# KarolinaBenkova/FEM-FCT-PDECO

Measured on AMD Instinct MI355X. Metric: FCT timesteps/sec (fwd+adj), higher is better.
Workload: dtype f64; 1 GPU; C2 advection_solidbody_FCT_PDECO_finaltime: [-1,1]^2 81x81 P1 (dx=0.025, n=6561), dt=1e-3, 250 fwd + 250 adj FCT steps per cost+gradient evaluation; nodes=6561, num_steps=250, batch_per_gpu=1, parallelism=single trajectory, low_order_solver=jacobi, jacobi_sweeps_max=26, graphs=True, graph_replay=True, kernel_regime=2

## Files before the change

fem-fct-pdeco_amd/csrc/ctx.hip:

```cpp
#include "femfct_internal.h"
#include "build_id.h"
#include "device_utils.h"

#include <dlfcn.h>
#include <stdarg.h>
#include <stdio.h>
#include <stdlib.h>
#include <string.h>
#include <algorithm>
#include <tuple>

int femfct_enqueue_artdiff(femfct_ctx* ctx, const double* K, double* D, int32_t batch);
int femfct_enqueue_spmv(femfct_ctx* ctx, const double* A, const double* x, double alpha, double beta, double* y,
                        int32_t batch);
int femfct_enqueue_cheb(femfct_ctx* ctx, const double* b, double* y_out, int iters, double lmin, double lmax,
                        int32_t batch, bool first_done_in_y1, const double* mdv = nullptr);
int femfct_mesh_release(femfct_ctx* ctx);
int femfct_build_structured_csr(femfct_ctx* ctx);

int femfct_fail(femfct_ctx* ctx, int code, const char* fmt, ...) {
    char buf[1024];
    va_list ap;
    va_start(ap, fmt);
    vsnprintf(buf, sizeof buf, fmt, ap);
    va_end(ap);
    if (ctx) ctx->err = buf;
    return code;
}

namespace {

__global__ void k_scatter_csr_to_ell(int64_t nnz, const int32_t* __restrict__ map, const double* __restrict__ v,
                                     double* __restrict__ ell) {
    int64_t k = (int64_t)blockIdx.x * blockDim.x + threadIdx.x;
    if (k < nnz) ell[map[k]] = v[k];
}

__global__ void k_gather_ell_to_csr(int64_t nnz, const int32_t* __restrict__ map, const double* __restrict__ ell,
                                    double* __restrict__ v) {
    int64_t k = (int64_t)blockIdx.x * blockDim.x + threadIdx.x;
    if (k < nnz) v[k] = ell[map[k]];
}

__global__ void k_mask_popcount(int64_t nbytes, const unsigned long long* __restrict__ mask, unsigned long long* __restrict__ out) {
    __shared__ unsigned long long s[256];
    unsigned long long c = 0;
    const int64_t words = nbytes >> 3;
    for (int64_t k = threadIdx.x; k < words; k += blockDim.x) c += (unsigned long long)__popcll(mask[k]);
    if (threadIdx.x == 0)
        for (int64_t k = words * 8; k < nbytes; ++k) c += (unsigned long long)__popc(reinterpret_cast<const uint8_t*>(mask)[k]);
    s[threadIdx.x] = c;
    __syncthreads();
    for (int o = 128; o > 0; o >>= 1) {
        if ((int)threadIdx.x < o) s[threadIdx.x] += s[threadIdx.x + o];
        __syncthreads();
    }
    if (threadIdx.x == 0) *out = s[0];
}

template <class T>
int dev_alloc(femfct_ctx* ctx, T** p, size_t count) {
    if (*p) { hipFree(*p); *p = nullptr; }
    if (count == 0) return FEMFCT_OK;
    hipError_t e = hipMalloc((void**)p, count * sizeof(T));
    if (e != hipSuccess) {
        *p = nullptr;
        return femfct_fail(ctx, FEMFCT_ERR_NOMEM, "hipMalloc(%zu bytes) failed: %s", count * sizeof(T),
                           hipGetErrorString(e));
    }
    return FEMFCT_OK;
}

template <class T>
void dev_free(T** p) {
    if (*p) hipFree(*p);
    *p = nullptr;
}

}

void femfct_release_pattern(femfct_ctx* ctx) {
    femfct_drop_graphs(ctx);
    dev_free(&ctx->d_cols); dev_free(&ctx->d_tslot); dev_free(&ctx->d_csr2ell); dev_free(&ctx->d_d2v);
    dev_free(&ctx->d_M); dev_free(&ctx->d_Ad); dev_free(&ctx->d_ml);
    dev_free(&ctx->d_L); dev_free(&ctx->d_D); dev_free(&ctx->d_F);
    dev_free(&ctx->d_b); dev_free(&ctx->d_xa); dev_free(&ctx->d_xb);
    dev_free(&ctx->d_du); dev_free(&ctx->d_y0); dev_free(&ctx->d_y1); dev_free(&ctx->d_y2); dev_free(&ctx->d_rdu);
    dev_free(&ctx->d_rp); dev_free(&ctx->d_rm); dev_free(&ctx->d_part); dev_free(&ctx->d_ctl);
    dev_free(&ctx->d_bigpart); ctx->bigpart_count = 0;
    dev_free(&ctx->d_Lmask);
    dev_free(&ctx->d_partk);
    dev_free(&ctx->d_zero);
    dev_free(&ctx->d_rot_check); ctx->rot_om_set = false;
    dev_free(&ctx->d_hA); dev_free(&ctx->d_hN); dev_free(&ctx->d_hrhs); dev_free(&ctx->d_hu);
    dev_free(&ctx->d_hout); dev_free(&ctx->d_hcsr);
    femfct_mesh_release(ctx);
    ctx->h_indptr.clear(); ctx->h_indices.clear(); ctx->h_csr2ell.clear(); ctx->h_cols.clear();
    dev_free(&ctx->d_trAall); ctx->trAall_count = 0;
    dev_free(&ctx->d_lowall); ctx->lowall_count = 0; ctx->low_src = nullptr;
    dev_free(&ctx->d_trA); dev_free(&ctx->d_trN); dev_free(&ctx->d_trRhs); dev_free(&ctx->d_level); dev_free(&ctx->d_log);
    dev_free(&ctx->d_ticket);
    ctx->tr_batch = 0; ctx->tr_steps = 0;
    dev_free(&ctx->d_scratch); ctx->scratch_count = 0;
    dev_free(&ctx->d_ttab); ctx->ttab_count = 0; ctx->h_ttab.clear();
    dev_free(&ctx->d_kry); dev_free(&ctx->d_kry_part); dev_free(&ctx->d_chs_om); dev_free(&ctx->d_chs_scale);
    ctx->chs_om_cap = 0;
    if (ctx->d_kry_ctl) { hipFree(ctx->d_kry_ctl); ctx->d_kry_ctl = nullptr; }
    if (ctx->d_kry_ctl2) { hipFree(ctx->d_kry_ctl2); ctx->d_kry_ctl2 = nullptr; }
    if (ctx->d_klog) { hipFree(ctx->d_klog); ctx->d_klog = nullptr; }
    ctx->kry_batch = 0;
    dev_free(&ctx->d_wscale); ctx->wscale_count = 0;
    dev_free(&ctx->d_zero_traj); ctx->zero_traj_count = 0;
    dev_free(&ctx->d_trMat); dev_free(&ctx->d_trBase); dev_free(&ctx->d_trBase2); dev_free(&ctx->d_trRhs2); dev_free(&ctx->d_trTmp);
    ctx->implicit_cols = false;
    ctx->n = 0; ctx->W = 0; ctx->nnz_csr = 0; ctx->ws_batch = 0; ctx->have_mass = false; ctx->structured = false; ctx->mass_is_mesh = false;
    ctx->sweep_budget = std::min(femfct_ctx().sweep_budget, ctx->max_iters);
    femfct_forget_jacobi_budgets(ctx);
}

void femfct_prof_begin(femfct_ctx* ctx, int cls) {
    if (!ctx->prof_on) return;
    femfct_ctx::ProfRec r;
    r.cls = cls;
    hipEventCreate(&r.a);
    hipEventCreate(&r.b);
    hipEventRecord(r.a, ctx->stream);
    ctx->prof.push_back(r);
}

void femfct_prof_end(femfct_ctx* ctx) {
    if (!ctx->prof_on || ctx->prof.empty()) return;
    hipEventRecord(ctx->prof.back().b, ctx->stream);
}

void femfct_drop_graphs(femfct_ctx* ctx) {
    for (auto& kv : ctx->graphs) hipGraphExecDestroy(kv.second);
    ctx->graphs.clear();
}

int femfct_ensure_workspace(femfct_ctx* ctx, int32_t batch) {
    if (ctx->solver == FEMFCT_SOLVER_BICGSTAB) {
        int rk = femfct_ensure_krylov_ws(ctx, batch);
        if (rk != FEMFCT_OK) return rk;
    }
#ifdef FEMFCT_TUNING
    if (!ctx->d_mesh_trace && getenv("FEMFCT_MESH_TRACE"))
        HIP_TRY(ctx, hipMalloc((void**)&ctx->d_mesh_trace, 16 * sizeof(unsigned long long)));
#endif
    if (!ctx->d_zero && ctx->n > 0) {
        int rz = dev_alloc(ctx, &ctx->d_zero, (size_t)ctx->n);
        if (rz != FEMFCT_OK) return rz;
        HIP_TRY(ctx, hipMemsetAsync(ctx->d_zero, 0, sizeof(double) * ctx->n, ctx->stream));
    }
    if (batch <= ctx->ws_batch) return FEMFCT_OK;
    femfct_drop_graphs(ctx);
    size_t nv = (size_t)batch * ctx->n, nm = nv * ctx->W;
    int rc;
#define A_(p, c) if ((rc = dev_alloc(ctx, &ctx->p, (c))) != FEMFCT_OK) return rc
    A_(d_L, nm + 1); A_(d_D, nm); A_(d_F, nm);
    HIP_TRY(ctx, hipMemsetAsync(ctx->d_L + nm, 0, sizeof(double), ctx->stream));
    A_(d_b, nv); A_(d_xa, nv); A_(d_xb, nv); A_(d_du, nv); A_(d_y0, nv); A_(d_y1, nv); A_(d_y2, nv);
    A_(d_rdu, nv); A_(d_rp, nv); A_(d_rm, nv);
    A_(d_part, (size_t)batch * 4 * FEMFCT_MAX_PARTIALS);
    A_(d_ctl, (size_t)batch);
    A_(d_partk, (size_t)batch * 16 * FEMFCT_MAX_PARTIALS);
    {
        const size_t words = ((size_t)batch * (size_t)ctx->n + 7) / 8 + 1;
        A_(d_Lmask, words);
        HIP_TRY(ctx, hipMemsetAsync(ctx->d_Lmask, 0, words * 8, ctx->stream));
    }
    {
        TilePlan tp;
        ctx->bigpart_count = 0;
        if (femfct_tile_plan(ctx, &tp, false) && femfct_tile_big(ctx, tp)) {
            ctx->bigpart_count = (int64_t)tp.tiles * tp.tiles;
            A_(d_bigpart, (size_t)batch * ctx->bigpart_count);
        }
    }
#undef A_
    HIP_TRY(ctx, hipMemsetAsync(ctx->d_ctl, 0, sizeof(StepCtl) * batch, ctx->stream));
    ctx->ws_batch = batch;
    return FEMFCT_OK;
}

static int fusion_mode(const femfct_ctx* ctx, int* K) {
    TilePlan tp;
    if (femfct_tile_plan(ctx, &tp, false)) {
        *K = tp.K;
        return femfct_tile_big(ctx, tp) ? 1 : 2;
    }
    StripPlan pl;
    if (femfct_strip_plan(ctx, &pl)) { *K = pl.K; return 1; }
    *K = 1;
    return 0;
}

int femfct_fused_k(const femfct_ctx* ctx) {
    int K;
    fusion_mode(ctx, &K);
    return K;
}

int femfct_next_budget(const femfct_ctx* ctx, int worst, bool coarse) {
    int K;
    const int mode = fusion_mode(ctx, &K);
    int b;
    if (mode == 2) b = std::max(worst, 1) + ((coarse || !ctx->exact_iters) ? 0 : 1);
    else if (mode == 1) b = std::max(worst, 1);
    else b = std::max(8, worst + worst / 8 + 2);
    return std::min(ctx->max_iters, b);
}

int femfct_grow_budget(const femfct_ctx* ctx, int budget) {
    int K;
    const int mode = fusion_mode(ctx, &K);
    if (mode == 2) return std::min(ctx->max_iters, budget + 2);
    if (mode == 1) return std::min(ctx->max_iters, budget + K);
    return std::min(ctx->max_iters, budget * 2);
}

int femfct_round_budget(const femfct_ctx* ctx, int b) {
    int K;
    if (fusion_mode(ctx, &K) == 0) b = (b + 3) & ~3;
    if (b < 1) b = 1;
    if (b > ctx->max_iters) b = ctx->max_iters;
    return b;
}

int femfct_install_pattern(femfct_ctx* ctx, int32_t n, int32_t W, const std::vector<int32_t>& cols,
                           const std::vector<uint8_t>& tslot) {
    int rc;
    ctx->n = n;
    ctx->W = W;
    if ((rc = dev_alloc(ctx, &ctx->d_cols, (size_t)W * n)) != FEMFCT_OK) return rc;
    if ((rc = dev_alloc(ctx, &ctx->d_tslot, (size_t)W * n)) != FEMFCT_OK) return rc;
    HIP_TRY(ctx, hipMemcpy(ctx->d_cols, cols.data(), sizeof(int32_t) * W * n, hipMemcpyHostToDevice));
    HIP_TRY(ctx, hipMemcpy(ctx->d_tslot, tslot.data(), sizeof(uint8_t) * W * n, hipMemcpyHostToDevice));
    if ((rc = dev_alloc(ctx, &ctx->d_M, (size_t)W * n)) != FEMFCT_OK) return rc;
    if ((rc = dev_alloc(ctx, &ctx->d_ml, (size_t)n)) != FEMFCT_OK) return rc;
    ctx->h_cols = cols;
    int32_t bwmax = 0;
    for (int32_t s = 1; s < W; ++s)
        for (int32_t i = 0; i < n; ++i) {
            int32_t d = cols[(size_t)s * n + i] - i;
            if (d < 0) d = -d;
            if (d > bwmax) bwmax = d;
        }
    ctx->bandwidth = bwmax;
    if (const char* e = getenv("FEMFCT_STRIPS")) ctx->use_strips = atoi(e) != 0;
    if (const char* e = getenv("FEMFCT_STRIP_K")) ctx->strip_k = atoi(e);
    if (const char* e = getenv("FEMFCT_TILES")) ctx->use_tiles = atoi(e) != 0;
    if (const char* e = getenv("FEMFCT_EXACT")) ctx->exact_iters = atoi(e) != 0;
    if (const char* e = getenv("FEMFCT_FUSE_BUILD")) ctx->fuse_build = atoi(e) != 0;
    if (const char* e = getenv("FEMFCT_PREASSEMBLE")) ctx->preassemble = atoi(e) != 0;
    if (const char* e = getenv("FEMFCT_PREASSEMBLE_MAX_GB")) ctx->preassemble_max_bytes = atof(e) * 1024.0 * 1024.0 * 1024.0;
    if (const char* e = getenv("FEMFCT_PREBUILD_LOW")) ctx->prebuild_low = atoi(e) != 0;
    if (const char* e = getenv("FEMFCT_WG_SLOTS")) ctx->wg_slots = std::max(1, atoi(e));
    if (const char* e = getenv("FEMFCT_DEEP_HALO")) ctx->deep_halo = atoi(e) != 0;
    if (const char* e = getenv("FEMFCT_FUSE_FLUX")) ctx->fuse_flux = atoi(e) != 0;
    if (const char* e = getenv("FEMFCT_FUSE_DUDT")) ctx->fuse_dudt = atoi(e) != 0;
    if (const char* e = getenv("FEMFCT_TILE_LEAN")) ctx->tile_lean = atoi(e) != 0;
    if (const char* e = getenv("FEMFCT_FUSE_END")) ctx->fuse_end = atoi(e) != 0;
    if (const char* e = getenv("FEMFCT_TILE4")) ctx->tile4_mode = atoi(e);
    if (const char* e = getenv("FEMFCT_LMASK")) ctx->l_mask = atoi(e) != 0;
    if (const char* e = getenv("FEMFCT_T4_XCD")) ctx->t4_xcd = atoi(e) != 0;
    if (const char* e = getenv("FEMFCT_T4_WALK")) ctx->t4_walk = atoi(e);
    if (const char* e = getenv("FEMFCT_T4_SNAKE")) ctx->t4_snake = atoi(e) != 0;
    if (const char* e = getenv("FEMFCT_T4_PAIR")) ctx->t4_pair = atoi(e) != 0;
#ifdef FEMFCT_TUNING
    if (const char* e = getenv("FEMFCT_PAIR_SHAPE")) ctx->pair_shape = atoi(e);
    if (const char* e = getenv("FEMFCT_PAIR_PRIO")) ctx->pair_prio = atoi(e);
    if (const char* e = getenv("FEMFCT_PAIR_SPLIT")) ctx->pair_split = std::min(90, std::max(10, atoi(e)));
    if (getenv("FEMFCT_PAIR_TRACE") && !ctx->d_pair_trace) {
        if (hipMalloc((void**)&ctx->d_pair_trace, sizeof(unsigned long long) * (FEMFCT_MAX_PARTIALS * 16 * 5 + 16)) == hipSuccess)
            hipMemset(ctx->d_pair_trace, 0, sizeof(unsigned long long) * (FEMFCT_MAX_PARTIALS * 16 * 5 + 16));
    }
    if (const char* e = getenv("FEMFCT_PAIR_STAGGER_US")) ctx->pair_stagger = (int)(atof(e) * 100.0);
#endif
    if (const char* e = getenv("FEMFCT_DEFER_CHECK")) ctx->defer_check = atoi(e) != 0;
    if (const char* e = getenv("FEMFCT_T4_INT")) ctx->t4_int = atoi(e) != 0;
    if (const char* e = getenv("FEMFCT_T4_WALKERS")) { int v = atoi(e); if (v > 0) ctx->num_cus = v; }
    if (const char* e = getenv("FEMFCT_INLINE_OPS")) ctx->inline_ops = atoi(e) != 0;
    if (const char* e = getenv("FEMFCT_HALF_D")) ctx->half_d = atoi(e) != 0;
    if (const char* e = getenv("FEMFCT_T4_STAGGER_US")) {
        const double us = atof(e);
        int pat = 7;
        if (const char* p = getenv("FEMFCT_T4_STAGGER_PAT")) pat = atoi(p);
        ctx->t4_stagger = us > 0 ? ((int)(us * 100.0) & 0xffffff) | ((pat & 15) << 24) : 0;
    }
    if (const char* e = getenv("FEMFCT_SINGLE_PATCH_BATCH")) { int v = atoi(e); ctx->single_patch_min_batch = v > 0 ? v : (1 << 30); }
    if (const char* e = getenv("FEMFCT_MESH_SOLVE")) ctx->mesh_solve = atoi(e) != 0;
    if (const char* e = getenv("FEMFCT_GEOM_MASS")) ctx->geom_mass = atoi(e) != 0;
    if (const char* e = getenv("FEMFCT_GEOM_ROT")) ctx->geom_rot = atoi(e) != 0;
    if (const char* e = getenv("FEMFCT_FORM_GROUPS")) ctx->form_groups = atoi(e) != 0;
    if (const char* e = getenv("FEMFCT_MESH_STEP")) ctx->mesh_step = atoi(e) != 0;
    if (const char* e = getenv("FEMFCT_MESH_STEP_BATCH")) ctx->mesh_step_min_batch = std::max(1, atoi(e));
    if (const char* e = getenv("FEMFCT_MESH_STEP_BATCH_LARGE")) ctx->mesh_step_min_batch_large = std::max(1, atoi(e));
    if (const char* e = getenv("FEMFCT_T4_DPP")) ctx->t4_dpp = atoi(e) != 0;
    if (const char* e = getenv("FEMFCT_T4_K")) ctx->t4_k = std::min(8, std::max(1, atoi(e)));
    if (const char* e = getenv("FEMFCT_SPECIES_SOLVER")) ctx->species_solver = atoi(e);
    if (const char* e = getenv("FEMFCT_STEPS_PER_GRAPH")) ctx->steps_per_graph = std::max(1, atoi(e));
    return femfct_strip_init(ctx);
}

static int build_csr_map(femfct_ctx* ctx) {
    const int32_t n = ctx->n, W = ctx->W;
    ctx->nnz_csr = ctx->h_indptr[n];
    ctx->h_csr2ell.assign(ctx->nnz_csr, 0);
    for (int32_t i = 0; i < n; ++i) {
        for (int32_t k = ctx->h_indptr[i]; k < ctx->h_indptr[i + 1]; ++k) {
            int32_t j = ctx->h_indices[k];
            int32_t s_found = -1;
            if (j == i) s_found = 0;
            else
                for (int32_t s = 1; s < W; ++s)
                    if (ctx->h_cols[(size_t)s * n + i] == j) { s_found = s; break; }
            if (s_found < 0) return femfct_fail(ctx, FEMFCT_ERR_INVALID, "CSR entry (%d,%d) not in the ELL pattern", i, j);
            ctx->h_csr2ell[k] = (int32_t)((size_t)s_found * n + i);
        }
    }
    int rc;
    if ((rc = dev_alloc(ctx, &ctx->d_csr2ell, (size_t)ctx->nnz_csr)) != FEMFCT_OK) return rc;
    HIP_TRY(ctx, hipMemcpy(ctx->d_csr2ell, ctx->h_csr2ell.data(), sizeof(int32_t) * ctx->nnz_csr, hipMemcpyHostToDevice));
    if ((rc = dev_alloc(ctx, &ctx->d_hcsr, (size_t)ctx->nnz_csr)) != FEMFCT_OK) return rc;
    return FEMFCT_OK;
}

extern "C" {

int femfct_abi_version(void) { return FEMFCT_ABI_VERSION; }
const char* femfct_build_id(void) { return FEMFCT_BUILD_ID; }

}

bool femfct_profiler_attached() {
    for (const char* name : {"librocprofiler-sdk.so.1", "librocprofiler-sdk.so"}) {
        if (void* h = dlopen(name, RTLD_LAZY | RTLD_NOLOAD)) {
            dlclose(h);
            return true;
        }
    }
    return false;
}

extern "C" {

int femfct_create(femfct_ctx** out, int device_id) {
    if (!out) return FEMFCT_ERR_INVALID;
    *out = nullptr;
    int count = 0;
    if (hipGetDeviceCount(&count) != hipSuccess || count <= 0) return FEMFCT_ERR_HIP;
    if (device_id < 0 || device_id >= count) return FEMFCT_ERR_INVALID;
    if (hipSetDevice(device_id) != hipSuccess) return FEMFCT_ERR_HIP;
    femfct_ctx* ctx = new (std::nothrow) femfct_ctx();
    if (!ctx) return FEMFCT_ERR_NOMEM;
    ctx->device = device_id;
    {
        int cus = 0;
        if (hipDeviceGetAttribute(&cus, hipDeviceAttributeMultiprocessorCount, device_id) == hipSuccess && cus > 0) ctx->num_cus = cus;
    }
    if (hipStreamCreateWithFlags(&ctx->stream, hipStreamNonBlocking) != hipSuccess) {
        delete ctx;
        return FEMFCT_ERR_HIP;
    }
    const char* pg = getenv("FEMFCT_PROFILER_GRAPHS");
    ctx->profiler_graphs_ok = pg && atoi(pg) != 0;
    if (!ctx->profiler_graphs_ok && femfct_profiler_attached()) ctx->graphs_blocked = true;
    *out = ctx;
    return FEMFCT_OK;
}

int femfct_graph_replay_active(const femfct_ctx* ctx, int* active_host) {
    if (!ctx || !active_host) return FEMFCT_ERR_INVALID;
    *active_host = (ctx->use_graphs && !ctx->prof_on && !ctx->graphs_blocked) ? 1 : 0;
    return FEMFCT_OK;
}

int femfct_rotation_derived(const femfct_ctx* ctx, int* derived_host) {
    if (!ctx || !derived_host) return FEMFCT_ERR_INVALID;
    *derived_host = ctx->last_rot_geom ? 1 : 0;
    return FEMFCT_OK;
}

int femfct_destroy(femfct_ctx* ctx) {
    if (!ctx) return FEMFCT_OK;
    hipSetDevice(ctx->device);
    hipStreamSynchronize(ctx->stream);
    if (ctx->d_pair_trace) {
        if (const char* path = getenv("FEMFCT_PAIR_TRACE")) {
            std::vector<unsigned long long> h((size_t)FEMFCT_MAX_PARTIALS * 16 * 5 + 16);
            if (hipMemcpy(h.data(), ctx->d_pair_trace, h.size() * sizeof(unsigned long long), hipMemcpyDeviceToHost) == hipSuccess)
                if (FILE* f = fopen(path, "wb")) { fwrite(h.data(), sizeof(unsigned long long), h.size(), f); fclose(f); }
        }
        hipFree(ctx->d_pair_trace);
        ctx->d_pair_trace = nullptr;
    }
    femfct_release_pattern(ctx);
    hipStreamDestroy(ctx->stream);
    delete ctx;
    return FEMFCT_OK;
}

const char* femfct_last_error(const femfct_ctx* ctx) { return ctx ? ctx->err.c_str() : "null context"; }

int femfct_synchronize(femfct_ctx* ctx) {
    FEMFCT_ENTER(ctx);
    ARG_TRY(ctx, ctx, "null ctx");
    HIP_TRY(ctx, hipStreamSynchronize(ctx->stream));
    return FEMFCT_OK;
}

void* femfct_stream(femfct_ctx* ctx) { return ctx ? (void*)ctx->stream : nullptr; }

int femfct_set_solver(femfct_ctx* ctx, int solver, double rel_tol, int max_iters) {
    FEMFCT_ENTER(ctx);
    ARG_TRY(ctx, ctx, "null ctx");
    ARG_TRY(ctx, solver == FEMFCT_SOLVER_JACOBI || solver == FEMFCT_SOLVER_BICGSTAB, "unknown solver");
    ARG_TRY(ctx, rel_tol > 0 && rel_tol < 1 && max_iters >= 1, "bad tolerance / iteration cap");
    ctx->solver = solver;
    ctx->solver_user = solver;
    femfct_forget_bicgstab_handovers(ctx);
    ctx->rel_tol = rel_tol;
    ctx->max_iters = max_iters;
    if (ctx->sweep_budget > max_iters) ctx->sweep_budget = max_iters;
    femfct_forget_jacobi_budgets(ctx);
    femfct_drop_graphs(ctx);
    return FEMFCT_OK;
}

int femfct_set_fusion(femfct_ctx* ctx, int strips, int tiles) {
    FEMFCT_ENTER(ctx);
    ARG_TRY(ctx, ctx, "null ctx");
    HIP_TRY(ctx, hipStreamSynchronize(ctx->stream));
    ctx->use_strips = strips != 0;
    ctx->use_tiles = tiles != 0;
    femfct_drop_graphs(ctx);
    femfct_forget_jacobi_budgets(ctx);
    ctx->ws_batch = 0;
    return FEMFCT_OK;
}

int femfct_kernel_regime(const femfct_ctx* ctx, int32_t batch) {
    if (!ctx || ctx->n <= 0) return -1;
    if (femfct_mesh_step_wanted(ctx, batch)) return FEMFCT_REGIME_MESH;
    if (femfct_tile4_wanted(ctx, batch)) return FEMFCT_REGIME_PATCH64;
    TilePlan tp;
    if (ctx->use_strips && femfct_tile_plan(ctx, &tp, true, 0, batch)) return FEMFCT_REGIME_TILE32;
    StripPlan sp;
    if (femfct_strip_plan(ctx, &sp)) return FEMFCT_REGIME_STRIPS;
    return FEMFCT_REGIME_ROWS;
}

int femfct_patch_walkers(const femfct_ctx* ctx, int32_t batch, int32_t sweeps) {
    if (!ctx || ctx->n <= 0 || batch < 1 || !femfct_tile4_wanted(ctx, batch) || femfct_single_patch(ctx, batch)) return 0;
    return femfct_tile4_walkers(ctx, femfct_tile4_halo(ctx, sweeps > 0 ? sweeps : 36), batch, false);
}

int femfct_launch_info(const femfct_ctx* ctx, int32_t* out4_host) {
    if (!ctx || !out4_host) return FEMFCT_ERR_INVALID;
    for (int k = 0; k < 4; ++k) out4_host[k] = ctx->last_launch[k];
    return FEMFCT_OK;
}

int femfct_lowop_nonzero_fraction(femfct_ctx* ctx, double* fraction_host) {
    FEMFCT_ENTER(ctx);
    ARG_TRY(ctx, fraction_host, "null argument");
    *fraction_host = 1.0;
    if (!ctx->d_Lmask || ctx->n <= 0 || !ctx->l_mask || !femfct_tile4_wanted(ctx, 1) || !ctx->t4_dpp ||
        ctx->solver != FEMFCT_SOLVER_JACOBI)
        return FEMFCT_OK;
    unsigned long long* d_cnt = nullptr;
    HIP_TRY(ctx, hipMalloc((void**)&d_cnt, sizeof(unsigned long long)));
    hipLaunchKernelGGL(k_mask_popcount, dim3(1), dim3(256), 0, ctx->stream, (int64_t)ctx->n, ctx->d_Lmask + 1, d_cnt);
    unsigned long long cnt = 0;
    HIP_TRY(ctx, hipMemcpyAsync(&cnt, d_cnt, sizeof cnt, hipMemcpyDeviceToHost, ctx->stream));
    HIP_TRY(ctx, hipStreamSynchronize(ctx->stream));
    hipFree(d_cnt);
    *fraction_host = (double)cnt / (6.0 * (double)ctx->n);
    return FEMFCT_OK;
}

int femfct_set_graphs(femfct_ctx* ctx, int enable) {
    FEMFCT_ENTER(ctx);
    ARG_TRY(ctx, ctx, "null ctx");
    ctx->use_graphs = enable != 0;
    if (!enable) femfct_drop_graphs(ctx);
    return FEMFCT_OK;
}

int femfct_set_profiling(femfct_ctx* ctx, int enable) {
    FEMFCT_ENTER(ctx);
    ARG_TRY(ctx, ctx, "null ctx");
    HIP_TRY(ctx, hipStreamSynchronize(ctx->stream));
    for (auto& r : ctx->prof) { hipEventDestroy(r.a); hipEventDestroy(r.b); }
    ctx->prof.clear();
    ctx->prof_on = enable != 0;
    return FEMFCT_OK;
}

int femfct_profile_report(femfct_ctx* ctx, double* total_ms_host, int32_t* launches_host, int32_t n_classes) {
    FEMFCT_ENTER(ctx);
    ARG_TRY(ctx, ctx && total_ms_host && launches_host && n_classes >= KC_COUNT, "need >= 8 classes");
    HIP_TRY(ctx, hipStreamSynchronize(ctx->stream));
    for (int k = 0; k < n_classes; ++k) { total_ms_host[k] = 0.0; launches_host[k] = 0; }
    for (auto& r : ctx->prof) {
        float ms = 0.f;
        if (hipEventElapsedTime(&ms, r.a, r.b) == hipSuccess) {
            total_ms_host[r.cls] += ms;
            launches_host[r.cls] += 1;
        }
        hipEventDestroy(r.a);
        hipEventDestroy(r.b);
    }
    ctx->prof.clear();
    return FEMFCT_OK;
}

int femfct_malloc(femfct_ctx* ctx, void** dev_ptr, size_t bytes) {
    FEMFCT_ENTER(ctx);
    ARG_TRY(ctx, ctx && dev_ptr, "null argument");
    HIP_TRY(ctx, hipSetDevice(ctx->device));
    hipError_t e = hipMalloc(dev_ptr, bytes ? bytes : 8);
    if (e != hipSuccess) return femfct_fail(ctx, FEMFCT_ERR_NOMEM, "hipMalloc(%zu) failed: %s", bytes, hipGetErrorString(e));
    return FEMFCT_OK;
}
int femfct_free(femfct_ctx* ctx, void* p) {
    FEMFCT_ENTER(ctx);
    ARG_TRY(ctx, ctx, "null ctx");
    HIP_TRY(ctx, hipStreamSynchronize(ctx->stream));
    HIP_TRY(ctx, hipFree(p));
    return FEMFCT_OK;
}
int femfct_memcpy_h2d(femfct_ctx* ctx, void* d, const void* h, size_t bytes) {
    FEMFCT_ENTER(ctx);
    ARG_TRY(ctx, ctx && (bytes == 0 || (d && h)), "null argument");
    HIP_TRY(ctx, hipMemcpyAsync(d, h, bytes, hipMemcpyHostToDevice, ctx->stream));
    HIP_TRY(ctx, hipStreamSynchronize(ctx->stream));
    return FEMFCT_OK;
}
int femfct_memcpy_d2h(femfct_ctx* ctx, void* h, const void* d, size_t bytes) {
    FEMFCT_ENTER(ctx);
    ARG_TRY(ctx, ctx && (bytes == 0 || (d && h)), "null argument");
    HIP_TRY(ctx, hipMemcpyAsync(h, d, bytes, hipMemcpyDeviceToHost, ctx->stream));
    HIP_TRY(ctx, hipStreamSynchronize(ctx->stream));
    return FEMFCT_OK;
}
int femfct_memcpy_d2d(femfct_ctx* ctx, void* d, const void* s, size_t bytes) {
    FEMFCT_ENTER(ctx);
    ARG_TRY(ctx, ctx && (bytes == 0 || (d && s)), "null argument");
    HIP_TRY(ctx, hipMemcpyAsync(d, s, bytes, hipMemcpyDeviceToDevice, ctx->stream));
    return FEMFCT_OK;
}
int femfct_memset0(femfct_ctx* ctx, void* d, size_t bytes) {
    FEMFCT_ENTER(ctx);
    ARG_TRY(ctx, ctx && (bytes == 0 || d), "null argument");
    HIP_TRY(ctx, hipMemsetAsync(d, 0, bytes, ctx->stream));
    return FEMFCT_OK;
}

int femfct_set_pattern_csr(femfct_ctx* ctx, int32_t n, const int32_t* indptr, const int32_t* indices) {
    FEMFCT_ENTER(ctx);
    ARG_TRY(ctx, ctx && indptr && indices && n > 0, "null/empty pattern");
    HIP_TRY(ctx, hipSetDevice(ctx->device));
    HIP_TRY(ctx, hipStreamSynchronize(ctx->stream));
    femfct_release_pattern(ctx);
    ARG_TRY(ctx, indptr[0] == 0, "indptr[0] must be 0");
    int32_t W = 1;
    for (int32_t i = 0; i < n; ++i) {
        ARG_TRY(ctx, indptr[i + 1] >= indptr[i], "indptr not monotone");
        int32_t len = 0;
        bool diag = false;
        for (int32_t k = indptr[i]; k < indptr[i + 1]; ++k) {
            int32_t j = indices[k];
            ARG_TRY(ctx, j >= 0 && j < n, "column index out of range");
            if (j == i) diag = true; else ++len;
        }
        ARG_TRY(ctx, diag, "pattern must contain the full diagonal");
        W = std::max(W, len + 1);
    }
    if (W > FEMFCT_MAX_W) return femfct_fail(ctx, FEMFCT_ERR_INVALID, "row with %d entries exceeds FEMFCT_MAX_W=%d", W, FEMFCT_MAX_W);
    std::vector<int32_t> cols((size_t)W * n);
    std::vector<uint8_t> tslot((size_t)W * n);
    for (int32_t s = 0; s < W; ++s)
        for (int32_t i = 0; i < n; ++i) { cols[(size_t)s * n + i] = i; tslot[(size_t)s * n + i] = (uint8_t)s; }
    for (int32_t i = 0; i < n; ++i) {
        int32_t s = 1;
        for (int32_t k = indptr[i]; k < indptr[i + 1]; ++k) {
            int32_t j = indices[k];
            if (j == i) continue;
            for (int32_t q = 1; q < s; ++q)
                ARG_TRY(ctx, cols[(size_t)q * n + i] != j, "duplicate column in a row");
            cols[(size_t)s * n + i] = j;
            ++s;
        }
    }
    for (int32_t i = 0; i < n; ++i)
        for (int32_t s = 1; s < W; ++s) {
            int32_t j = cols[(size_t)s * n + i];
            if (j == i) continue;
            int32_t ts = -1;
            for (int32_t q = 1; q < W; ++q)
                if (cols[(size_t)q * n + j] == i) { ts = q; break; }
            if (ts < 0) return femfct_fail(ctx, FEMFCT_ERR_INVALID, "pattern not symmetric: (%d,%d) has no transpose", i, j);
            tslot[(size_t)s * n + i] = (uint8_t)ts;
        }
    int rc = femfct_install_pattern(ctx, n, W, cols, tslot);
    if (rc != FEMFCT_OK) return rc;
    ctx->h_indptr.assign(indptr, indptr + n + 1);
    ctx->h_indices.assign(indices, indices + indptr[n]);
    return build_csr_map(ctx);
}

int32_t femfct_n(const femfct_ctx* ctx) { return ctx ? ctx->n : 0; }
int32_t femfct_ell_width(const femfct_ctx* ctx) { return ctx ? ctx->W : 0; }

int femfct_get_ell_cols(femfct_ctx* ctx, int32_t* cols_host) {
    FEMFCT_ENTER(ctx);
    ARG_TRY(ctx, ctx && cols_host && ctx->n > 0, "no pattern");
    memcpy(cols_host, ctx->h_cols.data(), sizeof(int32_t) * ctx->h_cols.size());
    return FEMFCT_OK;
}


static int need_csr_map(femfct_ctx* ctx) {
    ARG_TRY(ctx, ctx && ctx->n > 0, "no pattern registered");
    if (ctx->d_csr2ell) return FEMFCT_OK;
    if (ctx->structured) {
        int rc = femfct_build_structured_csr(ctx);
        if (rc != FEMFCT_OK) return rc;
        return build_csr_map(ctx);
    }
    return femfct_fail(ctx, FEMFCT_ERR_INVALID, "no CSR pattern");
}

int femfct_csr_to_ell(femfct_ctx* ctx, const double* csr_vals_host, double* ell_dev) {
    FEMFCT_ENTER(ctx);
    int rc = need_csr_map(ctx);
    if (rc != FEMFCT_OK) return rc;
    ARG_TRY(ctx, csr_vals_host && ell_dev, "null argument");
    HIP_TRY(ctx, hipMemcpyAsync(ctx->d_hcsr, csr_vals_host, sizeof(double) * ctx->nnz_csr, hipMemcpyHostToDevice, ctx->stream));
    HIP_TRY(ctx, hipMemsetAsync(ell_dev, 0, sizeof(double) * ctx->W * ctx->n, ctx->stream));
    int bs = 256;
    hipLaunchKernelGGL(k_scatter_csr_to_ell, dim3((unsigned)((ctx->nnz_csr + bs - 1) / bs)), dim3(bs), 0, ctx->stream,
                       ctx->nnz_csr, ctx->d_csr2ell, ctx->d_hcsr, ell_dev);
    HIP_TRY(ctx, hipStreamSynchronize(ctx->stream));
    return FEMFCT_OK;
}

int femfct_ell_to_csr(femfct_ctx* ctx, const double* ell_dev, double* csr_vals_host) {
    FEMFCT_ENTER(ctx);
    int rc = need_csr_map(ctx);
    if (rc != FEMFCT_OK) return rc;
    ARG_TRY(ctx, csr_vals_host && ell_dev, "null argument");
    int bs = 256;
    hipLaunchKernelGGL(k_gather_ell_to_csr, dim3((unsigned)((ctx->nnz_csr + bs - 1) / bs)), dim3(bs), 0, ctx->stream,
                       ctx->nnz_csr, ctx->d_csr2ell, ell_dev, ctx->d_hcsr);
    HIP_TRY(ctx, hipMemcpyAsync(csr_vals_host, ctx->d_hcsr, sizeof(double) * ctx->nnz_csr, hipMemcpyDeviceToHost, ctx->stream));
    HIP_TRY(ctx, hipStreamSynchronize(ctx->stream));
    return FEMFCT_OK;
}

int femfct_set_mass(femfct_ctx* ctx, const double* M_csr_vals_host, const double* ml_host) {
    FEMFCT_ENTER(ctx);
    ARG_TRY(ctx, ctx && ctx->n > 0, "no pattern registered");
    ARG_TRY(ctx, M_csr_vals_host && ml_host, "null argument");
    HIP_TRY(ctx, hipStreamSynchronize(ctx->stream));
    femfct_drop_graphs(ctx);
    int rc = femfct_csr_to_ell(ctx, M_csr_vals_host, ctx->d_M);
    if (rc != FEMFCT_OK) return rc;
    HIP_TRY(ctx, hipMemcpy(ctx->d_ml, ml_host, sizeof(double) * ctx->n, hipMemcpyHostToDevice));
    ctx->have_mass = true;
    ctx->mass_is_mesh = false;
    return FEMFCT_OK;
}

const double* femfct_mass_ell(const femfct_ctx* ctx) { return ctx && ctx->have_mass ? ctx->d_M : nullptr; }
const double* femfct_stiffness_ell(const femfct_ctx* ctx) { return ctx ? ctx->d_Ad : nullptr; }
const double* femfct_lumped_mass(const femfct_ctx* ctx) { return ctx && ctx->have_mass ? ctx->d_ml : nullptr; }

static int launch_step(femfct_ctx* ctx, const double* A, const double* N, int32_t nshared, const double* rhs,
                       const double* u_n, double dt, double* u_out, int32_t batch) {
    const int budget = femfct_round_budget(ctx, ctx->sweep_budget);
    femfct_ctx::GraphKey key{(uint64_t)1, key_bits(A), key_bits(N), key_bits(rhs), key_bits(u_n), key_bits(u_out),
                             key_bits(nshared), key_bits(batch), key_bits((int32_t)budget), key_bits(dt),
                             key_bits(ctx->rel_tol)};
    return femfct_run_graph(ctx, key, [&]() {
        return femfct_enqueue_step(ctx, A, N, nshared, rhs, u_n, dt, u_out, batch, budget);
    });
}

int femfct_fct_step(femfct_ctx* ctx, const double* A_ell, const double* N_ell, int32_t N_shared, const double* rhs,
                    const double* u_n, double dt, double* u_out, int32_t batch) {
    FEMFCT_ENTER(ctx);
    ARG_TRY(ctx, ctx && ctx->n > 0, "no pattern registered");
    ARG_TRY(ctx, ctx->have_mass, "mass matrix not set (femfct_set_mass / femfct_set_mesh_square)");
    ARG_TRY(ctx, A_ell && u_n && u_out, "null argument");
    ARG_TRY(ctx, batch >= 1 && dt > 0, "batch must be >= 1 and dt > 0");
    int rc = femfct_ensure_workspace(ctx, batch);
    if (rc != FEMFCT_OK) return rc;
    return launch_step(ctx, A_ell, N_ell, N_shared, rhs, u_n, dt, u_out, batch);
}

int femfct_last_step_info(femfct_ctx* ctx, femfct_step_info* info, int32_t batch) {
    FEMFCT_ENTER(ctx);
    ARG_TRY(ctx, ctx && info && batch >= 1 && batch <= ctx->ws_batch, "bad argument");
    std::vector<StepCtl> h(batch);
    HIP_TRY(ctx, hipMemcpyAsync(h.data(), ctx->d_ctl, sizeof(StepCtl) * batch, hipMemcpyDeviceToHost, ctx->stream));
    HIP_TRY(ctx, hipStreamSynchronize(ctx->stream));
    int worst = 0;
    for (int b = 0; b < batch; ++b) {
        info[b].flags = h[b].flags;
        info[b].solver_iters = h[b].iters;
        info[b].solver_resid = h[b].resid;
        info[b].min_rowsum = h[b].min_rowsum;
        worst = std::max(worst, h[b].iters);
    }
    bool short_of = false;
    for (int b = 0; b < batch; ++b) short_of = short_of || (h[b].flags & FEMFCT_FLAG_SOLVER_BUDGET);
    ctx->sweep_budget = short_of ? femfct_grow_budget(ctx, femfct_round_budget(ctx, ctx->sweep_budget))
                                 : femfct_next_budget(ctx, worst);
    return FEMFCT_OK;
}

int femfct_fct_step_host(femfct_ctx* ctx, const double* A_csr, const double* N_csr, const double* rhs,
                         const double* u_n, double dt, double* u_out, femfct_step_info* info) {
    FEMFCT_ENTER(ctx);
    ARG_TRY(ctx, ctx && ctx->n > 0, "no pattern registered");
    ARG_TRY(ctx, A_csr && u_n && u_out, "null argument");
    int rc;
    const size_t n = ctx->n, nm = n * ctx->W;
    if (!ctx->d_hA) {
        if ((rc = dev_alloc(ctx, &ctx->d_hA, nm)) != FEMFCT_OK) return rc;
        if ((rc = dev_alloc(ctx, &ctx->d_hN, nm)) != FEMFCT_OK) return rc;
        if ((rc = dev_alloc(ctx, &ctx->d_hrhs, n)) != FEMFCT_OK) return rc;
        if ((rc = dev_alloc(ctx, &ctx->d_hu, n)) != FEMFCT_OK) return rc;
        if ((rc = dev_alloc(ctx, &ctx->d_hout, n)) != FEMFCT_OK) return rc;
    }
    if ((rc = femfct_csr_to_ell(ctx, A_csr, ctx->d_hA)) != FEMFCT_OK) return rc;
    if (N_csr && (rc = femfct_csr_to_ell(ctx, N_csr, ctx->d_hN)) != FEMFCT_OK) return rc;
    if (rhs) HIP_TRY(ctx, hipMemcpyAsync(ctx->d_hrhs, rhs, sizeof(double) * n, hipMemcpyHostToDevice, ctx->stream));
    HIP_TRY(ctx, hipMemcpyAsync(ctx->d_hu, u_n, sizeof(double) * n, hipMemcpyHostToDevice, ctx->stream));
    femfct_step_info local;
    for (;;) {
        rc = femfct_fct_step(ctx, ctx->d_hA, N_csr ? ctx->d_hN : nullptr, 0, rhs ? ctx->d_hrhs : nullptr, ctx->d_hu,
                             dt, ctx->d_hout, 1);
        if (rc != FEMFCT_OK) return rc;
        const int used_budget = femfct_round_budget(ctx, ctx->sweep_budget);
        if ((rc = femfct_last_step_info(ctx, &local, 1)) != FEMFCT_OK) return rc;
        if (!(local.flags & FEMFCT_FLAG_SOLVER_BUDGET)) break;
        if (used_budget >= ctx->max_iters || !(local.solver_resid < INFINITY))
            return femfct_fail(ctx, FEMFCT_ERR_NOT_CONVERGED,
                               "low-order solve: residual %.3e after %d sweeps (tol %.1e)", local.solver_resid,
                               local.solver_iters, ctx->rel_tol);
        ctx->sweep_budget = femfct_grow_budget(ctx, used_budget);
    }
    if (info) *info = local;
    HIP_TRY(ctx, hipMemcpyAsync(u_out, ctx->d_hout, sizeof(double) * n, hipMemcpyDeviceToHost, ctx->stream));
    HIP_TRY(ctx, hipStreamSynchronize(ctx->stream));
    return FEMFCT_OK;
}

int femfct_chebsi(femfct_ctx* ctx, const double* b_dev, double* y_dev, int32_t cheb_iter, double lmin, double lmax,
                  int32_t batch) {
    FEMFCT_ENTER(ctx);
    ARG_TRY(ctx, ctx && ctx->n > 0 && ctx->have_mass, "mass matrix not set");
    ARG_TRY(ctx, b_dev && y_dev && cheb_iter >= 1 && batch >= 1 && lmin + lmax != 0, "bad argument");
    int rc = femfct_ensure_workspace(ctx, batch);
    if (rc != FEMFCT_OK) return rc;
    return femfct_enqueue_cheb(ctx, b_dev, y_dev, cheb_iter, lmin, lmax, batch, false);
}

int femfct_chebsi_md(femfct_ctx* ctx, const double* b_dev, double* y_dev, const double* md_dev, int32_t cheb_iter,
                     double lmin, double lmax, int32_t batch) {
    FEMFCT_ENTER(ctx);
    ARG_TRY(ctx, ctx && ctx->n > 0 && ctx->have_mass, "mass matrix not set");
    ARG_TRY(ctx, b_dev && y_dev && md_dev && cheb_iter >= 1 && batch == 1 && lmin + lmax != 0, "bad argument");
    int rc = femfct_ensure_workspace(ctx, batch);
    if (rc != FEMFCT_OK) return rc;
    return femfct_enqueue_cheb(ctx, b_dev, y_dev, cheb_iter, lmin, lmax, batch, false, md_dev);
}

int femfct_artificial_diffusion(femfct_ctx* ctx, const double* K_ell, double* D_ell, int32_t batch) {
    FEMFCT_ENTER(ctx);
    ARG_TRY(ctx, ctx && ctx->n > 0, "no pattern registered");
    ARG_TRY(ctx, K_ell && D_ell && batch >= 1, "bad argument");
    return femfct_enqueue_artdiff(ctx, K_ell, D_ell, batch);
}

int femfct_spmv(femfct_ctx* ctx, const double* mat_ell, const double* x_dev, double alpha, double beta, double* y_dev,
                int32_t batch) {
    FEMFCT_ENTER(ctx);
    ARG_TRY(ctx, ctx && ctx->n > 0, "no pattern registered");
    ARG_TRY(ctx, mat_ell && x_dev && y_dev && batch >= 1, "bad argument");
    return femfct_enqueue_spmv(ctx, mat_ell, x_dev, alpha, beta, y_dev, batch);
}

}
```

fem-fct-pdeco_amd/csrc/femfct_internal.h:

```cpp
#pragma once

#include <hip/hip_runtime.h>
#include <stdint.h>
#include <string.h>
#include <string>
#include <vector>
#include <map>
#include <tuple>

#include "../../include/femfct.h"

#define FEMFCT_MAX_W 16
#ifndef FEMFCT_MAX_PARTIALS
#define FEMFCT_MAX_PARTIALS 2048
#endif

struct StepCtl {
    int32_t flags;
    int32_t iters;
    int32_t done;
    int32_t parity;
    double  resid;
    double  bnorm;
    double  min_rowsum;
    double  rs[2];
    double  pad;
};

enum SweepKind {
    SWEEP_SOLIDBODY_FORWARD = 2, SWEEP_SOLIDBODY_ADJOINT = 3,
    SWEEP_NONLINEAR_FORWARD = 10, SWEEP_NONLINEAR_ADJOINT = 11,
    SWEEP_SCHNAK_FORWARD = 12, SWEEP_SCHNAK_ADJOINT = 13,
    SWEEP_CHTXS_FORWARD = 14, SWEEP_CHTXS_ADJOINT = 15,
    SWEEP_NONLINEAR_ADJOINT_ALLTIME = 16,
};

struct SweepKindState {
    int budget = 48;
    int good = 0;
    int fail = 0;
    int mesh_cap = 0;
    int cheb_budget = 40;
    int bicg_budget = 40;
    bool full_rows = false;
    bool low_bicg = false;
    bool cheb_off = false;
};

struct femfct_ctx {
    int device = 0;
    hipStream_t stream = nullptr;
    std::string err;

    int32_t n = 0;
    int32_t W = 0;
    int64_t nnz_csr = 0;
    int32_t* d_cols = nullptr;
    uint8_t* d_tslot = nullptr;
    int32_t* d_csr2ell = nullptr;
    std::vector<int32_t> h_indptr, h_indices, h_csr2ell, h_cols;
    bool structured = false;
    bool mass_is_mesh = false;
    double a1 = 0, a2 = 0, h = 0;
    int32_t n_cells = 0, N = 0, order = 0;
    int32_t* d_d2v = nullptr;

    double* d_M = nullptr;
    double* d_Ad = nullptr;
    double* d_ml = nullptr;
    bool have_mass = false;

    int solver = FEMFCT_SOLVER_JACOBI;
    int solver_user = FEMFCT_SOLVER_JACOBI;
    double rel_tol = 1e-13;
    int max_iters = 400;
    int sweep_budget = 48;
    std::map<int, SweepKindState> kinds;
    bool use_graphs = true;
    bool graphs_blocked = false;
    int graph_captures = 0;
    bool profiler_graphs_ok = false;
    int32_t steps_per_graph = 50;
    bool use_strips = true;
    bool use_tiles = true;
    bool mesh_solve = true;
    bool mesh_solve_attr[8] = {false, false, false, false, false, false, false, false};
    int single_patch_min_batch = 8;
    bool form_groups = true;
    bool geom_rot = true;
    double rot_om = 0.0;
    bool rot_om_set = false;
    int* d_rot_check = nullptr;
    bool last_rot_geom = false;
    bool geom_mass = true;
    bool t4_dpp = true;
    int t4_k = 8;
    int t4_snake = 1;
    bool t4_pair = true;
    int pair_stagger = 0;
    int32_t last_launch[4] = {0, 0, 0, 0};
    unsigned long long* d_pair_trace = nullptr;
    int pair_prio = 0, pair_split = 50;
    int pair_shape = 5;
    bool pair_rows = false;
    bool mesh_step = true;
    int mesh_step_min_batch = 1;
    int mesh_step_min_batch_large = 64;
    bool mesh_step_attr[6] = {false, false, false, false, false, false};
    double* d_zero = nullptr;
    unsigned long long* d_mesh_trace = nullptr;
    int defer_check = 1;
    int t4_int = 1;
    int t4_walk = 1;
    int num_cus = 256;
    int t4_xcd = 0;
    int t4_stagger = 600 | (7 << 24);
    int tile4_mode = 1;
    bool fuse_end = true;
    bool fuse_build = true;
    int wg_slots = 256;
    bool deep_halo = true;
    bool fuse_flux = true;
    bool fuse_dudt = true;
    int tile_lean = 1;
    bool exact_iters = false;
    int32_t bandwidth = 0;
    int32_t strip_k = 0;
    bool implicit_cols = false;

    int32_t ws_batch = 0;
    double *d_L = nullptr, *d_D = nullptr, *d_F = nullptr;
    double *d_b = nullptr, *d_xa = nullptr, *d_xb = nullptr;
    double *d_du = nullptr, *d_y0 = nullptr, *d_y1 = nullptr, *d_y2 = nullptr, *d_rdu = nullptr;
    double *d_rp = nullptr, *d_rm = nullptr;
    double *d_part = nullptr;
    StepCtl* d_ctl = nullptr;
    double* d_partk = nullptr;
    double* d_bigpart = nullptr;
    unsigned long long* d_Lmask = nullptr;
    bool half_d = true;
    bool inline_ops = true;
    bool l_mask = true;
    int64_t bigpart_count = 0;
    double *d_hA = nullptr, *d_hN = nullptr, *d_hrhs = nullptr, *d_hu = nullptr, *d_hout = nullptr, *d_hcsr = nullptr;

    typedef std::vector<uint64_t> GraphKey;
    std::map<GraphKey, hipGraphExec_t> graphs;

    int32_t tr_batch = 0, tr_steps = 0;
    double* d_trAall = nullptr;
    size_t trAall_count = 0;
    bool preassemble = true;
    double preassemble_max_bytes = 16.0 * 1024 * 1024 * 1024;
    bool prebuild_low = true;
    double* d_lowall = nullptr;
    size_t lowall_count = 0, low_doff = 0;
    const double* low_src = nullptr;
    double low_dt = 0.0;
    double *d_trA = nullptr, *d_trN = nullptr, *d_trRhs = nullptr;
    int32_t* d_level = nullptr;
    StepCtl* d_log = nullptr;
    unsigned* d_ticket = nullptr;
    int level_bias = 0, ord_bias = 0, rep_total = 1;
    bool rep_last = true;
    int end_req_delta = 0;
    bool end_req_krylov = false, end_fused = false;
    std::vector<StepCtl> h_log;
    int32_t log_steps = 0, log_batch = 0;

    bool prof_on = false;
    struct ProfRec { int cls; hipEvent_t a, b; };
    std::vector<ProfRec> prof;

    int32_t kry_batch = 0;
    double* d_kry = nullptr;
    double* d_kry_part = nullptr;
    void* d_kry_ctl = nullptr;
    void* d_kry_ctl2 = nullptr;
    double kry_tol = 1e-13;
    int kry_max_iters = 2000;
    int kry_budget = 40;
    void* d_klog = nullptr;
    int species_solver = 0;
    double* d_chs_om = nullptr;
    double* d_chs_scale = nullptr;
    int chs_om_cap = 0;
    std::vector<char> h_klog;
    double *d_trMat = nullptr, *d_trBase = nullptr, *d_trBase2 = nullptr;
    double *d_trRhs2 = nullptr, *d_trTmp = nullptr;
    double* d_wscale = nullptr;
    size_t wscale_count = 0;
    double* d_zero_traj = nullptr;
    size_t zero_traj_count = 0;

    double* d_scratch = nullptr;
    size_t scratch_count = 0;
    int32_t* d_ttab = nullptr;
    size_t ttab_count = 0;
    std::vector<int32_t> h_ttab;
};

int femfct_fail(femfct_ctx* ctx, int code, const char* fmt, ...);
#define HIP_TRY(ctx, expr)                                                          \
    do {                                                                            \
        hipError_t _e = (expr);                                                     \
        if (_e != hipSuccess)                                                       \
            return femfct_fail((ctx), FEMFCT_ERR_HIP, "%s failed: %s (%s:%d)", #expr, \
                               hipGetErrorString(_e), __FILE__, __LINE__);          \
    } while (0)
#define ARG_TRY(ctx, cond, msg)                                                     \
    do {                                                                            \
        if (!(cond)) return femfct_fail((ctx), FEMFCT_ERR_INVALID, "%s", msg);      \
    } while (0)

#define FEMFCT_ENTER(ctx)                                                           \
    do {                                                                            \
        if (!(ctx)) return FEMFCT_ERR_INVALID;                                      \
        HIP_TRY((ctx), hipSetDevice((ctx)->device));                                \
    } while (0)

int femfct_ensure_workspace(femfct_ctx* ctx, int32_t batch);
int femfct_ensure_krylov_ws(femfct_ctx* ctx, int32_t batch);
void femfct_drop_graphs(femfct_ctx* ctx);
void femfct_release_pattern(femfct_ctx* ctx);
int femfct_round_budget(const femfct_ctx* ctx, int b);
#define FEMFCT_INTERNAL __attribute__((visibility("hidden")))
FEMFCT_INTERNAL void femfct_forget_jacobi_budgets(femfct_ctx* ctx);
FEMFCT_INTERNAL void femfct_forget_bicgstab_handovers(femfct_ctx* ctx);
FEMFCT_INTERNAL void femfct_forget_cheb_off(femfct_ctx* ctx);
FEMFCT_INTERNAL int femfct_ensure_scratch(femfct_ctx* ctx, size_t doubles);
FEMFCT_INTERNAL void femfct_enqueue_reduce_levels(femfct_ctx* ctx, int32_t batch, int levels, int G, const double* partial,
                                                  int trapezoid, double scale, int accumulate, double* out_dev);

static inline uint64_t key_bits(const void* p) { return (uint64_t)(uintptr_t)p; }
static inline uint64_t key_bits(double d) { uint64_t u; memcpy(&u, &d, 8); return u; }
static inline uint64_t key_bits(int64_t v) { return (uint64_t)v; }
static inline uint64_t key_bits(int32_t v) { return (uint64_t)(int64_t)v; }
template <class F>
int femfct_run_graph(femfct_ctx* ctx, const femfct_ctx::GraphKey& key, F&& enqueue);

static inline bool femfct_tiles_usable(const femfct_ctx* ctx) {
    return ctx->use_strips && ctx->use_tiles && ctx->implicit_cols && ctx->W == 7;
}

struct StripPlan { int K, R, bw, rpt, S; };
bool femfct_strip_plan(const femfct_ctx* ctx, StripPlan* pl);
int femfct_strip_init(femfct_ctx* ctx);
int femfct_enqueue_strip_jacobi(femfct_ctx* ctx, const StripPlan& pl, const double* L, const double* b, double* xa,
                                double* xb, int launch, int g_build, int32_t batch);
int femfct_enqueue_strip_cheb(femfct_ctx* ctx, const StripPlan& pl, const double* b, const double* in_mid,
                              const double* in_old, double* y_out, int k_first, int k_last, const double* omegas,
                              double md_scale, double* bufA0, double* bufA1, double* bufB0, double* bufB1,
                              int32_t batch);

struct TilePlan { int tiles, K, H; };
bool femfct_tile_plan(const femfct_ctx* ctx, TilePlan* pl, bool need_partials = true, int budget = 0, int batch = 1);
bool femfct_tile_big(const femfct_ctx* ctx, const TilePlan& pl);
bool femfct_cheb_flux_fusable(const femfct_ctx* ctx, int32_t batch);
bool femfct_geom_mass(const femfct_ctx* ctx);
int femfct_enqueue_tile_build_jacobi(femfct_ctx* ctx, const TilePlan& pl, struct MatRef A, const double* Nm, int32_t nshared,
                                     struct VecRef rhs, int64_t rhs_bstride, struct VecRef u_n, int64_t u_bstride, double dt,
                                     int32_t batch, bool pre = false);
int femfct_enqueue_low_seq(femfct_ctx* ctx, const double* A, double* L, double* D, int32_t entries, double dt);
int femfct_enqueue_tile_jacobi(femfct_ctx* ctx, const TilePlan& pl, const double* L, const double* b, double* xa,
                               double* xb, int launch, int g_build, int32_t batch, bool last, int bn_launch = 0, int defer = 0);
__attribute__((visibility("hidden"))) void femfct_launch_reduce_resid(femfct_ctx* ctx, int64_t count, int launch, int32_t batch);
int femfct_enqueue_tile_dudt_cheb(femfct_ctx* ctx, struct MatRef A, struct VecRef rhs, int64_t rhs_bstride, double* ulow,
                                  int budget_units, int part_count, int iters_per_unit, int exact_k, int iters,
                                  const double* omegas, double md_scale, int32_t batch, int* tail_first = nullptr);
int femfct_enqueue_tile_cheb(femfct_ctx* ctx, const TilePlan& pl, const double* b, const double* in_mid,
                             const double* in_old, double* y_out, int k_first, int k_last, const double* omegas,
                             double md_scale, double* bufA0, double* bufA1, double* bufB0, double* bufB1, int32_t batch,
                             const struct ChebIO* io = nullptr);
int femfct_enqueue_tile_cheb_flux_limit(femfct_ctx* ctx, const double* b, const double* in_mid, const double* in_old,
                                        int k_first, int k_last, const double* omegas, double md_scale, struct MatRef D,
                                        const double* ulow, double dt, struct VecRef out, int64_t out_bstride, int32_t batch,
                                        bool fuse_end);
int femfct_enqueue_tile_flux_limit(femfct_ctx* ctx, const double* D, const double* ulow, const double* du, double dt,
                                   struct VecRef out, int64_t out_bstride, int32_t batch, bool* fuse_end_io, int half_d = 0);

bool femfct_tile4_wanted(const femfct_ctx* ctx, int32_t batch);
bool femfct_single_patch(const femfct_ctx* ctx, int32_t batch);
int femfct_tile4_tiles(const femfct_ctx* ctx, int H = 8);
int femfct_tile4_halo(const femfct_ctx* ctx, int sweeps);
int femfct_tile4_walkers(const femfct_ctx* ctx, int H, int32_t batch, bool pair);
bool femfct_jacobi_pair_wanted(const femfct_ctx* ctx, int H, int32_t batch, bool have_lmask, bool assume_upwind_rows = false);
int femfct_tile4_init(femfct_ctx* ctx);
int femfct_enqueue_tile4_jacobi(femfct_ctx* ctx, const double* L, const double* b, double* xa, double* xb, int launch,
                                int g_build, int32_t batch, int H = 8, int K = 8, int check_every = 0,
                                const uint8_t* lmask = nullptr);
int femfct_enqueue_tile4_cheb(femfct_ctx* ctx, const double* b, const double* in_mid, const double* in_old, double* y_out,
                              int k_first, int k_last, const double* omegas, double md_scale, double* bufA0, double* bufA1,
                              double* bufB0, double* bufB1, int32_t batch,
                              const struct ChebIO* io = nullptr);

bool femfct_rotation_is_geometric(femfct_ctx* ctx, const double* Arot, double* om_out);
bool femfct_jacobi_plan(const femfct_ctx* ctx, int budget, int batch, int* K, int* launches);
bool femfct_mesh_step_wanted(const femfct_ctx* ctx, int32_t batch, bool have_nm = false);
int femfct_enqueue_mesh_step(femfct_ctx* ctx, struct MatRef A, const double* Nm, int32_t nshared, struct VecRef rhs,
                             int64_t rhs_bstride, struct VecRef u_n, int64_t u_bstride, double dt, struct VecRef u_out,
                             int64_t out_bstride, int32_t batch, int32_t budget, bool fuse_end);
int femfct_fused_k(const femfct_ctx* ctx);
int femfct_next_budget(const femfct_ctx* ctx, int worst_iters, bool coarse = false);
int femfct_grow_budget(const femfct_ctx* ctx, int budget);

enum { KC_BUILD_LOW = 0, KC_JACOBI, KC_DUDT_RHS, KC_CHEB, KC_FLUX, KC_LIMIT, KC_ASSEMBLE, KC_OTHER, KC_COUNT };
void femfct_prof_begin(femfct_ctx* ctx, int cls);
void femfct_prof_end(femfct_ctx* ctx);

struct LaunchGeom { dim3 grid; dim3 block; };
LaunchGeom femfct_geom(const femfct_ctx* ctx, int32_t batch);

int femfct_enqueue_step(femfct_ctx* ctx, const double* A, const double* N, int32_t nshared,
                        const double* rhs, const double* u_n, double dt, double* u_out,
                        int32_t batch, int32_t budget);

bool femfct_profiler_attached();

template <class F>
int femfct_run_graph(femfct_ctx* ctx, const femfct_ctx::GraphKey& key, F&& enqueue) {
    if (!ctx->use_graphs || ctx->prof_on || ctx->graphs_blocked) return enqueue();
    auto it = ctx->graphs.find(key);
    if (it == ctx->graphs.end()) {
        if (!ctx->profiler_graphs_ok && femfct_profiler_attached()) {
            ctx->graphs_blocked = true;
            return enqueue();
        }
        if (ctx->graphs.size() > 64) femfct_drop_graphs(ctx);
        ++ctx->graph_captures;
        hipGraph_t graph = nullptr;
        HIP_TRY(ctx, hipStreamBeginCapture(ctx->stream, hipStreamCaptureModeThreadLocal));
        int rc = enqueue();
        hipError_t e = hipStreamEndCapture(ctx->stream, &graph);
        if (rc != FEMFCT_OK) { if (graph) hipGraphDestroy(graph); return rc; }
        if (e != hipSuccess) return femfct_fail(ctx, FEMFCT_ERR_HIP, "hipStreamEndCapture: %s", hipGetErrorString(e));
        hipGraphExec_t exec = nullptr;
        e = hipGraphInstantiate(&exec, graph, nullptr, nullptr, 0);
        hipGraphDestroy(graph);
        if (e != hipSuccess) return femfct_fail(ctx, FEMFCT_ERR_HIP, "hipGraphInstantiate: %s", hipGetErrorString(e));
        it = ctx->graphs.emplace(key, exec).first;
    }
    HIP_TRY(ctx, hipGraphLaunch(it->second, ctx->stream));
    return FEMFCT_OK;
}
```

fem-fct-pdeco_amd/csrc/kernels_tile32.hip:

```cpp
#include "femfct_internal.h"
#include "device_utils.h"
#include "solve_ctl.h"
#include "forms.h"
#include "step_end.h"
#include "sweep_common.h"

#include <math.h>

#define TILE_T 16
#define TILE_H 8
#define TILE_L 32
#define TILE_LD 33
#define TILE_HMAX 13

namespace {

struct TileGeom {
    int lx, ly, gx, gy, i;
    bool inside, owned;
    int kvalid;
    int nb[6];
    int self;
};

template <int T = TILE_T, int H = TILE_H, int PL = TILE_L>
__device__ __forceinline__ TileGeom tile_geom(int N) {
    static_assert(T + 2 * H == PL, "patch edge = tile + 2 halos");
    constexpr int PLD = PL + 1;
    TileGeom g;
    g.lx = threadIdx.x % PL;
    g.ly = threadIdx.x / PL;
    const int x0 = blockIdx.x * T - H, y0 = blockIdx.y * T - H;
    g.gx = x0 + g.lx;
    g.gy = y0 + g.ly;
    g.inside = g.gx >= 0 && g.gx < N && g.gy >= 0 && g.gy < N;
    g.i = g.inside ? g.gy * N + g.gx : 0;
    g.owned = g.inside && g.lx >= H && g.lx < H + T && g.ly >= H && g.ly < H + T;
    int kv = 1 << 20;
    if (x0 > 0) kv = min(kv, g.lx);
    if (x0 + PL - 1 < N - 1) kv = min(kv, PL - 1 - g.lx);
    if (y0 > 0) kv = min(kv, g.ly);
    if (y0 + PL - 1 < N - 1) kv = min(kv, PL - 1 - g.ly);
    g.kvalid = g.inside ? kv : 0;
    const int dx[6] = {1, 1, 0, -1, -1, 0}, dy[6] = {0, 1, 1, 0, -1, -1};
    g.self = g.ly * PLD + g.lx;
#pragma unroll
    for (int s = 0; s < 6; ++s) {
        int nx = min(max(g.lx + dx[s], 0), PL - 1), ny = min(max(g.ly + dy[s], 0), PL - 1);
        g.nb[s] = ny * PLD + nx;
    }
    return g;
}

template <int H>
__device__ __forceinline__ int tile_dist(const TileGeom& g) {
    constexpr int T = TILE_L - 2 * H;
    const int ddx = max(max(H - g.lx, g.lx - (H + T - 1)), 0), ddy = max(max(H - g.ly, g.ly - (H + T - 1)), 0);
    return max(ddx, ddy);
}

struct LeanAddr {
    const double* n0[6];
    double* me0;
};

__device__ __forceinline__ LeanAddr lean_addr(double (*bufs)[TILE_L * TILE_LD], const TileGeom& g) {
    LeanAddr a;
    a.me0 = &bufs[0][g.self];
#pragma unroll
    for (int s = 0; s < 6; ++s) a.n0[s] = &bufs[0][g.nb[s]];
    return a;
}

template <int BUF, int LAST>
__device__ __forceinline__ void lean_jacobi_sweep(const LeanAddr& a, bool live, bool owned, const double* lv, double dg,
                                                  double rdg, double bv, double& xo, double& rmax) {
    constexpr int RD = BUF * TILE_L * TILE_LD, WR = (1 - BUF) * TILE_L * TILE_LD;
    if (live) {
        double acc = bv;
#pragma unroll
        for (int s = 0; s < 6; ++s) acc = fma(-lv[s], a.n0[s][RD], acc);
        if (LAST && owned) rmax = nan_max(rmax, fabs(acc - dg * xo));
        xo = acc * rdg;
        a.me0[WR] = xo;
    }
    __syncthreads();
}

__device__ __forceinline__ double lean_jacobi(const LeanAddr& a, int klive, int K, bool owned, const double* lv, double dg,
                                              double rdg, double bv, double xi, double& rmax) {
    double xo = xi;
    int k = 0;
    for (; k + 2 < K; k += 2) {
        lean_jacobi_sweep<0, 0>(a, k < klive, owned, lv, dg, rdg, bv, xo, rmax);
        lean_jacobi_sweep<1, 0>(a, k + 1 < klive, owned, lv, dg, rdg, bv, xo, rmax);
    }
    if (k + 1 < K) {
        lean_jacobi_sweep<0, 0>(a, k < klive, owned, lv, dg, rdg, bv, xo, rmax);
        lean_jacobi_sweep<1, 1>(a, k + 1 < klive, owned, lv, dg, rdg, bv, xo, rmax);
    } else if (k < K) {
        lean_jacobi_sweep<0, 1>(a, k < klive, owned, lv, dg, rdg, bv, xo, rmax);
    }
    return xo;
}

template <int BUF>
__device__ __forceinline__ void lean_cheb_iter(const LeanAddr& a, bool live, const double* mv, double md, double rmd, double bv,
                                               double wk, double& ym, double& yo) {
    constexpr int RD = BUF * TILE_L * TILE_LD, WR = (1 - BUF) * TILE_L * TILE_LD;
    if (live) {
        double acc = md * ym;
#pragma unroll
        for (int s = 0; s < 6; ++s) acc = fma(mv[s], a.n0[s][RD], acc);
        const double z = (bv - acc) * rmd;
        const double yn = wk * (z + ym - yo) + yo;
        yo = ym;
        ym = yn;
        a.me0[WR] = yn;
    }
    __syncthreads();
}

template <int H, int EXACT, int BIG, int LEAN>
__global__ void __launch_bounds__(STRIP_T)
k_tile_jacobi(int n, int N, const double* __restrict__ L_, const double* __restrict__ b_, double* __restrict__ xa_,
              double* __restrict__ xb_, double* __restrict__ part, StepCtl* __restrict__ ctl_, int launch, int K,
              int g_build, double rel_tol, double* __restrict__ bigpart, double* __restrict__ partk, int bn_launch,
              int defer) {
    constexpr int W = 7;
    __shared__ double xs[2][TILE_L * TILE_LD];
    __shared__ double smem[96];
    const int bz = blockIdx.z;
    StepCtl* ctl = ctl_ + bz;
    if (!defer && ctl->done) return;
    double* p = part + (int64_t)bz * 4 * FEMFCT_MAX_PARTIALS;
    const int nwg = gridDim.x * gridDim.y, wg = blockIdx.y * gridDim.x + blockIdx.x;
    double bnorm;
    double rmax_prev = 0.0;
    bool have_rmax = false;
    if (defer) {
        bnorm = 0.0;
    } else if (launch == bn_launch) {
        double rsmin = INFINITY;
        bnorm = 0.0;
        if (!BIG && launch > 0 && g_build == nwg) {
            const double* pr = p + ((launch - 1) & 1) * FEMFCT_MAX_PARTIALS;
            for (int k = threadIdx.x; k < nwg; k += blockDim.x) {
                bnorm = nan_max(bnorm, p[2 * FEMFCT_MAX_PARTIALS + k]);
                rmax_prev = nan_max(rmax_prev, pr[k]);
                rsmin = nan_min(rsmin, p[3 * FEMFCT_MAX_PARTIALS + k]);
            }
            block_reduce_max_max_min(bnorm, rmax_prev, rsmin, smem);
            have_rmax = true;
        } else {
            bnorm = reduce_partials(p + 2 * FEMFCT_MAX_PARTIALS, g_build, OpMax(), 0.0, smem);
            rsmin = reduce_partials(p + 3 * FEMFCT_MAX_PARTIALS, g_build, OpMin(), INFINITY, smem);
        }
        if (wg == 0 && threadIdx.x == 0) {
            ctl->bnorm = bnorm;
            ctl->min_rowsum = rsmin;
            if (!(rsmin > 0.0)) ctl->flags |= FEMFCT_FLAG_MMATRIX_ROWSUM;
        }
    } else {
        bnorm = ctl->bnorm;
    }
    if (launch > 0 && !defer) {
        double rmax = have_rmax ? rmax_prev
                      : BIG   ? ctl->rs[(launch - 1) & 1]
                              : reduce_partials(p + ((launch - 1) & 1) * FEMFCT_MAX_PARTIALS, nwg, OpMax(), 0.0, smem);
        if (rmax <= rel_tol * bnorm) {
            if (wg == 0 && threadIdx.x == 0) {
                ctl->done = 1; ctl->parity = launch & 1; ctl->iters = launch * K; ctl->flags |= FEMFCT_FLAG_COARSE_ITERS;
                ctl->resid = bnorm != 0.0 ? rmax / bnorm : 0.0;
            }
            return;
        }
    }
    const int64_t moff = (int64_t)bz * W * n, voff = (int64_t)bz * n;
    const double* L = L_ + moff;
    const double* xin = ((launch & 1) ? xb_ : xa_) + voff;
    double* xout = ((launch & 1) ? xa_ : xb_) + voff;
    const TileGeom g = tile_geom<TILE_L - 2 * H, H>(N);
    double lv[W - 1], dg = 1.0, rdg = 1.0, bv = 0.0, xi = 0.0;
#pragma unroll
    for (int s = 0; s < W - 1; ++s) lv[s] = 0.0;
    if (g.inside) {
        dg = L[g.i];
        rdg = 1.0 / dg;
#pragma unroll
        for (int s = 1; s < W; ++s) lv[s - 1] = L[(int64_t)s * n + g.i];
        bv = b_[voff + g.i];
        xi = xin[g.i];
    }
    xs[0][g.self] = xi;
    if (LEAN) xs[1][g.self] = xi;
    __syncthreads();
    double rmax = 0.0;
    int cur = 0;
    [[maybe_unused]] double xo = xi;
    [[maybe_unused]] const int klive = min(g.kvalid, K - tile_dist<H>(g));
    [[maybe_unused]] const LeanAddr a = lean_addr(xs, g);
    if (!EXACT) {
        if constexpr (LEAN) xo = lean_jacobi(a, klive, K, g.owned, lv, dg, rdg, bv, xi, rmax);
        else
        for (int k = 0; k < K; ++k) {
            const double* c = xs[cur];
            double xn = c[g.self];
            if (k < g.kvalid) {
                double acc = bv;
#pragma unroll
                for (int s = 0; s < W - 1; ++s) acc = fma(-lv[s], c[g.nb[s]], acc);
                if (k == K - 1 && g.owned) rmax = nan_max(rmax, fabs(acc - dg * xn));
                xn = acc * rdg;
            }
            xs[cur ^ 1][g.self] = xn;
            __syncthreads();
            cur ^= 1;
        }
    } else {
        double rk[H];
#pragma unroll
        for (int k = 0; k < H; ++k) {
            rk[k] = 0.0;
            if (k < K) {
                if constexpr (LEAN) {
                    const int rd = (k & 1) * TILE_L * TILE_LD, wr = ((k + 1) & 1) * TILE_L * TILE_LD;
                    if (k < klive) {
                        double acc = bv;
#pragma unroll
                        for (int s = 0; s < W - 1; ++s) acc = fma(-lv[s], a.n0[s][rd], acc);
                        if (g.owned) rk[k] = fabs(acc - dg * xo);
                        if (k == K - 1) rmax = nan_max(rmax, rk[k]);
                        xo = acc * rdg;
                        a.me0[wr] = xo;
                    }
                    __syncthreads();
                    continue;
                }
                const double* c = xs[cur];
                double xn = c[g.self];
                if (k < g.kvalid) {
                    double acc = bv;
#pragma unroll
                    for (int s = 0; s < W - 1; ++s) acc = fma(-lv[s], c[g.nb[s]], acc);
                    if (g.owned) rk[k] = fabs(acc - dg * xn);
                    if (k == K - 1) rmax = nan_max(rmax, rk[k]);
                    xn = acc * rdg;
                }
                xs[cur ^ 1][g.self] = xn;
                __syncthreads();
                cur ^= 1;
            }
        }
        __shared__ double sk[H][STRIP_T / WAVE];
        const int wid = threadIdx.x / WAVE, lane = threadIdx.x % WAVE;
#pragma unroll
        for (int k = 0; k < H; ++k) {
            double v = wave_reduce(rk[k], OpMax());
            if (lane == 0) sk[k][wid] = v;
        }
        __syncthreads();
        if (threadIdx.x < H) {
            double v = 0.0;
            for (int w = 0; w < STRIP_T / WAVE; ++w) v = nan_max(v, sk[threadIdx.x][w]);
            partk[((int64_t)bz * 16 + threadIdx.x) * FEMFCT_MAX_PARTIALS + wg] = v;
        }
    }
    if (g.owned) xout[g.i] = LEAN ? xo : xs[cur][g.self];
    rmax = block_reduce(rmax, OpMax(), 0.0, smem);
    if (threadIdx.x == 0) {
        if (BIG) bigpart[(int64_t)bz * nwg + wg] = rmax;
        else if (defer) partk[((int64_t)bz * 16 + launch) * FEMFCT_MAX_PARTIALS + wg] = rmax;
        else p[(launch & 1) * FEMFCT_MAX_PARTIALS + wg] = rmax;
    }
}

template <int H, int PRE, int LEAN>
__global__ void __launch_bounds__(STRIP_T)
k_tile_build_jacobi(int n, int N, MatRef A_ref, const double* __restrict__ N_, int nshared,
                    VecRef rhs_ref, int64_t rhs_bstride, VecRef u_ref, int64_t u_bstride,
                    const double* __restrict__ ml, double dt, double* __restrict__ L_, double* __restrict__ D_,
                    double* __restrict__ b_, double* __restrict__ xb_, double* __restrict__ part,
                    StepCtl* __restrict__ ctl_, int K) {
    constexpr int W = 7;
    __shared__ double xs[2][TILE_L * TILE_LD];
    __shared__ double as[PRE ? 1 : 3][TILE_L * TILE_LD];
    __shared__ double smem[96];
    const int bz = blockIdx.z;
    const int wg = blockIdx.y * gridDim.x + blockIdx.x;
    double* p = part + (int64_t)bz * 4 * FEMFCT_MAX_PARTIALS;
    if (wg == 0 && threadIdx.x == 0) {
        StepCtl* c = ctl_ + bz;
        c->flags = 0; c->iters = 0; c->done = 0; c->parity = 0; c->resid = 0.0; c->bnorm = 0.0;
        c->min_rowsum = 0.0;
    }
    const int64_t moff = (int64_t)bz * W * n, voff = (int64_t)bz * n;
    const double* A = mat_ptr(A_ref, bz);
    const double* Nm = N_ ? N_ + (nshared ? 0 : moff) : nullptr;
    const double* rhs = vec_ptr(rhs_ref);
    if (rhs) rhs += bz * rhs_bstride;
    const double* u = vec_ptr(u_ref) + bz * u_bstride;
    const TileGeom g = tile_geom<TILE_L - 2 * H, H>(N);
    double lv[W - 1], dv[W - 1], dsum = 0.0, rs = 0.0;
    double dg = 1.0, rdg = 1.0, bv = 0.0, xi = 0.0;
    if constexpr (PRE) {
#pragma unroll
        for (int s = 0; s < W - 1; ++s) lv[s] = 0.0;
        if (g.inside) {
            dg = A[g.i];
#pragma unroll
            for (int s = 1; s < W; ++s) lv[s - 1] = A[(int64_t)s * n + g.i];
        }
#pragma unroll
        for (int s = 0; s < W - 1; ++s) rs += lv[s];
        if (g.inside) {
            const double mli = ml[g.i];
            rs += dg;
            rdg = 1.0 / dg;
            xi = u[g.i];
            bv = mli * xi + (rhs ? dt * rhs[g.i] : 0.0);
        }
    } else {
        const int dx[6] = {1, 1, 0, -1, -1, 0}, dy[6] = {0, 1, 1, 0, -1, -1};
        bool ex[W - 1];
#pragma unroll
        for (int s = 0; s < W - 1; ++s) {
            const int nx = g.gx + dx[s], ny = g.gy + dy[s];
            ex[s] = g.inside && nx >= 0 && nx < N && ny >= 0 && ny < N;
        }
        double av[W - 1], at[W - 1], a0 = 0.0;
#pragma unroll
        for (int s = 0; s < W - 1; ++s) av[s] = 0.0;
        if (g.inside) {
            a0 = A[g.i];
#pragma unroll
            for (int s = 1; s < W; ++s) av[s - 1] = A[(int64_t)s * n + g.i];
        }
#pragma unroll
        for (int s = 0; s < 3; ++s) as[s][g.self] = av[s + 3];
        __syncthreads();
#pragma unroll
        for (int s = 0; s < 3; ++s) at[s] = as[s][g.nb[s]];
        __syncthreads();
#pragma unroll
        for (int s = 0; s < 3; ++s) as[s][g.self] = av[s];
        __syncthreads();
#pragma unroll
        for (int s = 3; s < 6; ++s) at[s] = as[s - 3][g.nb[s]];
#pragma unroll
        for (int s = 0; s < W - 1; ++s) {
            const double a = av[s];
            const double d = ex[s] ? fmax(0.0, fmax(a, at[s])) : 0.0;
            dsum += d;
            double l = dt * (a - d);
            if (Nm && g.inside) l += dt * Nm[(int64_t)(s + 1) * n + g.i];
            lv[s] = l;
            dv[s] = d;
            rs += l;
        }
        if (g.inside) {
            const double mli = ml[g.i];
            double ld = mli + dt * (a0 + dsum);
            if (Nm) ld += dt * Nm[g.i];
            rs += ld;
            dg = ld;
            rdg = 1.0 / dg;
            xi = u[g.i];
            bv = mli * xi + (rhs ? dt * rhs[g.i] : 0.0);
        }
    }
    double bmax = 0.0, rsmin = INFINITY;
    if (g.owned) {
        double* L = L_ + moff;
        L[g.i] = dg;
#pragma unroll
        for (int s = 1; s < W; ++s) L[(int64_t)s * n + g.i] = lv[s - 1];
        if constexpr (!PRE) {
            double* D = D_ + moff;
            D[g.i] = -dsum;
#pragma unroll
            for (int s = 1; s < W; ++s) D[(int64_t)s * n + g.i] = dv[s - 1];
        }
        b_[voff + g.i] = bv;
        bmax = fabs(bv);
        rsmin = rs;
    }
    xs[0][g.self] = xi;
    if (LEAN) xs[1][g.self] = xi;
    __syncthreads();
    double rmax = 0.0;
    int cur = 0;
    [[maybe_unused]] double xo = xi;
    if constexpr (LEAN) xo = lean_jacobi(lean_addr(xs, g), min(g.kvalid, K - tile_dist<H>(g)), K, g.owned, lv, dg, rdg, bv, xi, rmax);
    else
    for (int k = 0; k < K; ++k) {
        const double* c = xs[cur];
        double xn = c[g.self];
        if (k < g.kvalid) {
            double acc = bv;
#pragma unroll
            for (int s = 0; s < W - 1; ++s) acc = fma(-lv[s], c[g.nb[s]], acc);
            if (k == K - 1 && g.owned) rmax = nan_max(rmax, fabs(acc - dg * xn));
            xn = acc * rdg;
        }
        xs[cur ^ 1][g.self] = xn;
        __syncthreads();
        cur ^= 1;
    }
    if (g.owned) xb_[voff + g.i] = LEAN ? xo : xs[cur][g.self];
    block_reduce_max_max_min(rmax, bmax, rsmin, smem);
    if (threadIdx.x == 0) {
        p[wg] = rmax;
        p[2 * FEMFCT_MAX_PARTIALS + wg] = bmax;
        p[3 * FEMFCT_MAX_PARTIALS + wg] = rsmin;
    }
}

__global__ void __launch_bounds__(256)
k_low_seq(int n, int N, const double* __restrict__ A_, const double* __restrict__ ml, double dt, double* __restrict__ L_,
          double* __restrict__ D_) {
    constexpr int W = 7;
    const int64_t off = (int64_t)blockIdx.y * W * n;
    const double* A = A_ + off;
    double* L = L_ + off;
    double* D = D_ + off;
    const int dx[6] = {1, 1, 0, -1, -1, 0}, dy[6] = {0, 1, 1, 0, -1, -1};
    for (int i = blockIdx.x * blockDim.x + threadIdx.x; i < n; i += gridDim.x * blockDim.x) {
        const int gx = i % N, gy = i / N;
        double av[W - 1], at[W - 1];
        bool ex[W - 1];
        const double a0 = A[i];
#pragma unroll
        for (int s = 0; s < W - 1; ++s) {
            const int nx = gx + dx[s], ny = gy + dy[s];
            ex[s] = nx >= 0 && nx < N && ny >= 0 && ny < N;
            av[s] = A[(int64_t)(s + 1) * n + i];
            at[s] = ex[s] ? A[(int64_t)(s < 3 ? s + 4 : s - 2) * n + ny * N + nx] : 0.0;
        }
        double dsum = 0.0;
#pragma unroll
        for (int s = 0; s < W - 1; ++s) {
            const double a = av[s];
            const double d = ex[s] ? fmax(0.0, fmax(a, at[s])) : 0.0;
            dsum += d;
            L[(int64_t)(s + 1) * n + i] = dt * (a - d);
            D[(int64_t)(s + 1) * n + i] = d;
        }
        L[i] = ml[i] + dt * (a0 + dsum);
        D[i] = -dsum;
    }
}

__global__ void __launch_bounds__(STRIP_T)
k_reduce_resid(const double* __restrict__ bigpart, int64_t count, StepCtl* __restrict__ ctl_, int launch) {
    __shared__ double smem[32];
    const int bz = blockIdx.x;
    if (ctl_[bz].done) return;
    const double* q = bigpart + (int64_t)bz * count;
    double v = 0.0;
    for (int64_t k = threadIdx.x; k < count; k += blockDim.x) v = nan_max(v, q[k]);
    v = block_reduce(v, OpMax(), 0.0, smem);
    if (threadIdx.x == 0) ctl_[bz].rs[launch & 1] = v;
}

template <int H, int LEAN>
__global__ void __launch_bounds__(STRIP_T)
k_tile_cheb(int n, int N, const double* __restrict__ M, const double* __restrict__ b_, const double* __restrict__ ymid_,
            const double* __restrict__ yold_, double* __restrict__ omid_, double* __restrict__ oold_, int K,
            CheOmegas om, double md_scale, ChebIO cio) {
    constexpr int W = 7;
    __shared__ double ys[LEAN ? 2 : 3][TILE_L * TILE_LD];
    const int64_t voff = (int64_t)blockIdx.z * n;
    if (cio.mat) M = cio.mat + (int64_t)blockIdx.z * cio.mat_bs;
    if (cio.scale_dev) md_scale = cio.scale_dev[blockIdx.z];
    const double* omd = cio.om_dev ? cio.om_dev + (int64_t)blockIdx.z * cio.om_bs + cio.k0 : nullptr;
    if (cio.mid_ref.base) ymid_ = vec_ptr(cio.mid_ref) + (int64_t)blockIdx.z * cio.mid_bs - voff;
    if (cio.out_ref.base) omid_ = const_cast<double*>(vec_ptr(cio.out_ref)) + (int64_t)blockIdx.z * cio.out_bs - voff;
    const TileGeom g = tile_geom<TILE_L - 2 * H, H>(N);
    double mv[W - 1], md = 1.0, rmd = 1.0, bv = 0.0, ym = 0.0, yo = 0.0;
#pragma unroll
    for (int s = 0; s < W - 1; ++s) mv[s] = 0.0;
    if (g.inside) {
        md = M[g.i];
        rmd = 1.0 / (md_scale * md);
#pragma unroll
        for (int s = 1; s < W; ++s) mv[s - 1] = M[(int64_t)s * n + g.i];
        bv = b_[voff + g.i];
        if (ymid_) ym = ymid_[voff + g.i];
        if (yold_) yo = yold_[voff + g.i];
    }
    if constexpr (LEAN) {
        ys[0][g.self] = ym;
        ys[1][g.self] = ym;
        __syncthreads();
        const int klive = min(g.kvalid, K - tile_dist<H>(g));
        const LeanAddr a = lean_addr(ys, g);
        int k = 0;
        for (; k + 1 < K; k += 2) {
            lean_cheb_iter<0>(a, k < klive, mv, md, rmd, bv, omd ? omd[k] : om.w[k], ym, yo);
            lean_cheb_iter<1>(a, k + 1 < klive, mv, md, rmd, bv, omd ? omd[k + 1] : om.w[k + 1], ym, yo);
        }
        if (k < K) lean_cheb_iter<0>(a, k < klive, mv, md, rmd, bv, omd ? omd[k] : om.w[k], ym, yo);
        if (g.owned) {
            omid_[voff + g.i] = ym;
            if (oold_) oold_[voff + g.i] = yo;
        }
        return;
    }
    ys[0][g.self] = yo;
    ys[1][g.self] = ym;
    __syncthreads();
    int io = 0, im = 1, in_ = 2;
    for (int k = 0; k < K; ++k) {
        const double* ymd = ys[im];
        const double ymv = ymd[g.self];
        double yn = ymv;
        if (k < g.kvalid) {
            double acc = md * ymv;
#pragma unroll
            for (int s = 0; s < W - 1; ++s) acc = fma(mv[s], ymd[g.nb[s]], acc);
            const double z = (bv - acc) * rmd;
            const double yov = ys[io][g.self];
            const double wk = omd ? omd[k] : om.w[k];
            yn = wk * (z + ymv - yov) + yov;
        }
        ys[in_][g.self] = yn;
        __syncthreads();
        int t = io; io = im; im = in_; in_ = t;
    }
    if (g.owned) {
        omid_[voff + g.i] = ys[im][g.self];
        if (oold_) oold_[voff + g.i] = ys[io][g.self];
    }
}


#define FL_H 2
template <int PL>
__device__ __forceinline__ int fl_nb(int s) {
    const int lx = threadIdx.x % PL, ly = threadIdx.x / PL;
    const int dx = (s == 0 || s == 1) ? 1 : (s == 3 || s == 4) ? -1 : 0;
    const int dy = (s == 1 || s == 2) ? 1 : (s == 4 || s == 5) ? -1 : 0;
    return min(max(ly + dy, 0), PL - 1) * (PL + 1) + min(max(lx + dx, 0), PL - 1);
}

template <int FL_L, int GEOM, int HALFD>
__global__ void __launch_bounds__(FL_L * FL_L, FL_L == 32 ? 8 : 1)
k_tile_flux_limit(int n, int N, double h, const double* __restrict__ M, const double* __restrict__ D_,
                  const double* __restrict__ ulow_, const double* __restrict__ du_, const double* __restrict__ ml,
                  double dt, VecRef out_ref, int64_t out_bstride, EndArgs e) {
    constexpr int W = 7;
    constexpr int FL_LD = FL_L + 1, FL_T = FL_L - 2 * FL_H;
    __shared__ double su[FL_L * FL_LD], sd[FL_L * FL_LD], srp[FL_L * FL_LD], srm[FL_L * FL_LD];
    __shared__ double sdf[HALFD ? 3 : 1][HALFD ? FL_L * FL_LD : 1];
    if (FL_L == 16) step_log_early(e);
    const int bz = blockIdx.z;
    const int64_t moff = (int64_t)bz * W * n, voff = (int64_t)bz * n;
    const TileGeom g = tile_geom<FL_T, FL_H, FL_L>(N);
    double ui = 0.0, dui = 0.0, mli = 1.0, dfw[3] = {0.0, 0.0, 0.0};
    if (g.inside) { ui = ulow_[voff + g.i]; dui = du_[voff + g.i]; mli = ml[g.i]; }
    if (HALFD) {
        if (g.inside) {
#pragma unroll
            for (int s = 0; s < 3; ++s) dfw[s] = D_[moff + (int64_t)(s + 1) * n + g.i];
        }
#pragma unroll
        for (int s = 0; s < 3; ++s) sdf[s][g.self] = dfw[s];
    }
    su[g.self] = ui;
    sd[g.self] = dui;
    srp[g.self] = 1.0;
    srm[g.self] = 1.0;
    __syncthreads();
    double f[W - 1];
    const bool have = g.inside && g.kvalid >= 1;
    if (have) {
        double pp = 0.0, pm = 0.0, umax = ui, umin = ui;
        const int pc = (GEOM || HALFD) ? mass_edge_counts(g.gx, g.gy, N - 1) : 0;
        const double mq = (0.5 * h * h) / 12.0;
#pragma unroll
        for (int s = 1; s < W; ++s) {
            const int64_t idx = (int64_t)s * n + g.i;
            const int nbs = fl_nb<FL_L>(s - 1);
            const double uj = su[nbs];
            const double mij = GEOM ? (double)((pc >> (2 * (s - 1))) & 3) * mq : M[idx];
            double dij;
            if (HALFD) {
                const bool exists = ((pc >> (2 * (s - 1))) & 3) != 0;
                dij = s <= 3 ? sdf[s - 1][g.self] : (exists ? sdf[s - 4][nbs] : 0.0);
            } else {
                dij = D_[moff + idx];
            }
            const double fs = mij * (dui - sd[nbs]) + dij * (ui - uj);
            f[s - 1] = fs;
            pp += fmax(fs, 0.0);
            pm += fmin(fs, 0.0);
            const bool live = (mij != 0.0) || (dij != 0.0);
            umax = live ? fmax(umax, uj) : umax;
            umin = live ? fmin(umin, uj) : umin;
        }
        const double qp = umax - ui, qm = umin - ui;
        srp[g.self] = (pp != 0.0) ? fmin(1.0, mli * qp / (dt * pp)) : 1.0;
        srm[g.self] = (pm != 0.0) ? fmin(1.0, mli * qm / (dt * pm)) : 1.0;
    }
    __syncthreads();
    if (g.owned) {
        const double rpi = srp[g.self], rmi = srm[g.self];
        double fbar = 0.0;
#pragma unroll
        for (int s = 0; s < W - 1; ++s) {
            const double fs = f[s];
            const int nbs = fl_nb<FL_L>(s);
            const double a = (fs > 0.0) ? fmin(rpi, srm[nbs]) : fmin(rmi, srp[nbs]);
            fbar += a * fs;
        }
        double* out = const_cast<double*>(vec_ptr(out_ref)) + bz * out_bstride;
        out[g.i] = ui + dt * fbar / mli;
    }
    if (FL_L == 16) step_end_by_last_workgroup(e);
}

template <int GEOM, int LEAN>
__global__ void __launch_bounds__(STRIP_T, LEAN ? 8 : 1)
k_tile_cheb_flux_limit(int n, int N, double h, const double* __restrict__ M, const double* __restrict__ b_,
                       const double* __restrict__ ymid_, const double* __restrict__ yold_, int K, CheOmegas om,
                       double md_scale, MatRef D_ref, const double* __restrict__ ulow_,
                       const double* __restrict__ ml, double dt, VecRef out_ref, int64_t out_bstride, EndArgs e) {
    constexpr int W = 7, HH = 12;
    __shared__ double ys[LEAN ? 2 : 3][TILE_L * TILE_LD];
    __shared__ double su[TILE_L * TILE_LD], srp[TILE_L * TILE_LD], srm[TILE_L * TILE_LD];
    const int bz = blockIdx.z;
    const int64_t voff = (int64_t)bz * n;
    const double* D_ = mat_ptr(D_ref, bz);
    const TileGeom g = tile_geom<TILE_L - 2 * HH, HH>(N);
    double mv[W - 1], dv[W - 1], md = 1.0, rmd = 1.0, bv = 0.0, ym = 0.0, yo = 0.0, ui = 0.0, mli = 1.0;
#pragma unroll
    for (int s = 0; s < W - 1; ++s) { mv[s] = 0.0; dv[s] = 0.0; }
    if (g.inside) {
        md = M[g.i];
        rmd = 1.0 / (md_scale * md);
        if (GEOM) {
            const int pc = mass_edge_counts(g.gx, g.gy, N - 1);
            const double mq = (0.5 * h * h) / 12.0;
#pragma unroll
            for (int s = 1; s < W; ++s) mv[s - 1] = (double)((pc >> (2 * (s - 1))) & 3) * mq;
        } else {
#pragma unroll
            for (int s = 1; s < W; ++s) mv[s - 1] = M[(int64_t)s * n + g.i];
        }
        bv = b_[voff + g.i];
        ym = ymid_[voff + g.i];
        yo = yold_[voff + g.i];
        ui = ulow_[voff + g.i];
        mli = ml[g.i];
    }
    ys[0][g.self] = LEAN ? ym : yo;
    ys[1][g.self] = ym;
    su[g.self] = ui;
    srp[g.self] = 1.0;
    srm[g.self] = 1.0;
    __syncthreads();
    step_log_early(e);
    if (g.inside) {
#pragma unroll
        for (int s = 1; s < W; ++s) dv[s - 1] = D_[(int64_t)s * n + g.i];
    }
    int io = 0, im = 1, in_ = 2;
    const bool have = g.inside && g.kvalid >= K + 1 && (!LEAN || tile_dist<HH>(g) <= 1);
    if constexpr (LEAN) {
        const int klive = min(g.kvalid, K - max(tile_dist<HH>(g) - 2, 0));
        const LeanAddr a = lean_addr(ys, g);
        int k = 0;
        for (; k + 1 < K; k += 2) {
            lean_cheb_iter<0>(a, k < klive, mv, md, rmd, bv, om.w[k], ym, yo);
            lean_cheb_iter<1>(a, k + 1 < klive, mv, md, rmd, bv, om.w[k + 1], ym, yo);
        }
        if (k < K) lean_cheb_iter<0>(a, k < klive, mv, md, rmd, bv, om.w[k], ym, yo);
        im = K & 1;
    } else
    for (int k = 0; k < K; ++k) {
        const double* ymd = ys[im];
        const double ymv = ymd[g.self];
        double yn = ymv;
        if (k < g.kvalid) {
            double acc = md * ymv;
#pragma unroll
            for (int s = 0; s < W - 1; ++s) acc = fma(mv[s], ymd[g.nb[s]], acc);
            const double z = (bv - acc) * rmd;
            const double yov = ys[io][g.self];
            yn = om.w[k] * (z + ymv - yov) + yov;
        }
        ys[in_][g.self] = yn;
        __syncthreads();
        int t = io; io = im; im = in_; in_ = t;
    }
    const double* sd = ys[im];
    const double dui = LEAN ? ym : sd[g.self];
    double f[W - 1];
    if (have) {
        double pp = 0.0, pm = 0.0, umax = ui, umin = ui;
#pragma unroll
        for (int s = 0; s < W - 1; ++s) {
            const double uj = su[g.nb[s]];
            const double mij = mv[s], dij = dv[s];
            const double fs = mij * (dui - sd[g.nb[s]]) + dij * (ui - uj);
            f[s] = fs;
            pp += fmax(fs, 0.0);
            pm += fmin(fs, 0.0);
            const bool live = (mij != 0.0) || (dij != 0.0);
            umax = live ? fmax(umax, uj) : umax;
            umin = live ? fmin(umin, uj) : umin;
        }
        const double qp = umax - ui, qm = umin - ui;
        srp[g.self] = (pp != 0.0) ? fmin(1.0, mli * qp / (dt * pp)) : 1.0;
        srm[g.self] = (pm != 0.0) ? fmin(1.0, mli * qm / (dt * pm)) : 1.0;
    }
    __syncthreads();
    if (g.owned) {
        const double rpi = srp[g.self], rmi = srm[g.self];
        double fbar = 0.0;
#pragma unroll
        for (int s = 0; s < W - 1; ++s) {
            const double fs = f[s];
            const double a = (fs > 0.0) ? fmin(rpi, srm[g.nb[s]]) : fmin(rmi, srp[g.nb[s]]);
            fbar += a * fs;
        }
        double* out = const_cast<double*>(vec_ptr(out_ref)) + bz * out_bstride;
        out[g.i] = ui + dt * fbar / mli;
    }
    step_end_by_last_workgroup(e);
}

template <int LEAN>
__global__ void __launch_bounds__(STRIP_T)
k_tile_dudt_cheb(int n, int N, MatRef A_ref, VecRef rhs_ref, int64_t rhs_bstride,
                 const double* __restrict__ M, const double* __restrict__ xa_, const double* __restrict__ xb_,
                 double* __restrict__ ulow_, double* __restrict__ rdu_, double* __restrict__ omid_,
                 double* __restrict__ oold_, double* __restrict__ part, StepCtl* __restrict__ ctl_, int budget,
                 int part_count, int iters_per_unit, double rel_tol, const double* __restrict__ partk, int exact_k,
                 int K, CheOmegas om, double md_scale, double omega1) {
    constexpr int W = 7, H = 10;
    __shared__ double ys[LEAN ? 2 : 3][TILE_L * TILE_LD];
    __shared__ double smem[64];
    const int bz = blockIdx.z;
    StepCtl* ctl = ctl_ + bz;
    double* p = part + (int64_t)bz * 4 * FEMFCT_MAX_PARTIALS;
    const int wg = blockIdx.y * gridDim.x + blockIdx.x;
    if (exact_k < 0 && blockIdx.y == gridDim.x) {
        if (blockIdx.x == 0)
            deferred_test_publish(ctl, deferred_test_load(p, partk + (int64_t)bz * 16 * FEMFCT_MAX_PARTIALS, part_count, -exact_k),
                                  -exact_k, iters_per_unit, rel_tol);
        return;
    }
    const int parity = exact_k < 0 ? (budget & 1) : ctl->done ? ctl->parity : (budget & 1);
    if (exact_k >= 0)
        finalize_solve(ctl, p, part_count, budget, iters_per_unit, rel_tol, smem,
                       partk ? partk + (int64_t)bz * 16 * FEMFCT_MAX_PARTIALS : nullptr, exact_k, wg == 0);
    const int64_t voff = (int64_t)bz * n;
    const double* A = mat_ptr(A_ref, bz);
    const double* x = (parity ? xb_ : xa_) + voff;
    const double* rhs = vec_ptr(rhs_ref);
    if (rhs) rhs += bz * rhs_bstride;
    const TileGeom g = tile_geom<TILE_L - 2 * H, H>(N);
    double av[W], mv[W - 1], md = 1.0, rmd = 1.0, ui = 0.0, ri = 0.0;
#pragma unroll
    for (int s = 0; s < W; ++s) av[s] = 0.0;
#pragma unroll
    for (int s = 0; s < W - 1; ++s) mv[s] = 0.0;
    if (g.inside) {
        md = M[g.i];
        rmd = 1.0 / (md_scale * md);
#pragma unroll
        for (int s = 0; s < W; ++s) av[s] = A[(int64_t)s * n + g.i];
#pragma unroll
        for (int s = 1; s < W; ++s) mv[s - 1] = M[(int64_t)s * n + g.i];
        ui = x[g.i];
        ri = rhs ? rhs[g.i] : 0.0;
    }
    constexpr int UB = LEAN ? 0 : 2;
    ys[UB][g.self] = ui;
    __syncthreads();
    double r = 0.0, y1 = 0.0;
    if (g.kvalid >= 1) {
        double acc = av[0] * ui;
#pragma unroll
        for (int s = 1; s < W; ++s) acc = fma(av[s], ys[UB][g.nb[s - 1]], acc);
        r = -acc + ri;
        y1 = omega1 * (r / (md_scale * md));
    }
    if constexpr (LEAN) {
        ys[1][g.self] = y1;
        __syncthreads();
        ys[0][g.self] = y1;
        double ym = y1, yo = 0.0;
        const int dist = tile_dist<H>(g);
        const LeanAddr a = lean_addr(ys, g);
        auto live = [&](int k) { return k + 1 < g.kvalid && k < K - dist; };
        int k = 0;
        for (; k + 1 < K; k += 2) {
            lean_cheb_iter<1>(a, live(k), mv, md, rmd, r, om.w[k], ym, yo);
            lean_cheb_iter<0>(a, live(k + 1), mv, md, rmd, r, om.w[k + 1], ym, yo);
        }
        if (k < K) lean_cheb_iter<1>(a, live(k), mv, md, rmd, r, om.w[k], ym, yo);
        if (g.owned) {
            ulow_[voff + g.i] = ui;
            rdu_[voff + g.i] = r;
            omid_[voff + g.i] = ym;
            if (oold_) oold_[voff + g.i] = yo;
        }
        return;
    }
    __syncthreads();
    ys[0][g.self] = 0.0;
    ys[1][g.self] = y1;
    __syncthreads();
    int io = 0, im = 1, in_ = 2;
    for (int k = 0; k < K; ++k) {
        const double* ymd = ys[im];
        const double ymv = ymd[g.self];
        double yn = ymv;
        if (k + 1 < g.kvalid) {
            double acc = md * ymv;
#pragma unroll
            for (int s = 0; s < W - 1; ++s) acc = fma(mv[s], ymd[g.nb[s]], acc);
            const double z = (r - acc) * rmd;
            const double yov = ys[io][g.self];
            yn = om.w[k] * (z + ymv - yov) + yov;
        }
        ys[in_][g.self] = yn;
        __syncthreads();
        int t = io; io = im; im = in_; in_ = t;
    }
    if (g.owned) {
        ulow_[voff + g.i] = ui;
        rdu_[voff + g.i] = r;
        omid_[voff + g.i] = ys[im][g.self];
        if (oold_) oold_[voff + g.i] = ys[io][g.self];
    }
}

}


int femfct_enqueue_tile_build_jacobi(femfct_ctx* ctx, const TilePlan& pl, MatRef A, const double* Nm, int32_t nshared,
                                     VecRef rhs, int64_t rhs_bstride, VecRef u_n, int64_t u_bstride, double dt,
                                     int32_t batch, bool pre) {
    if (pre && Nm) return femfct_fail(ctx, FEMFCT_ERR_INVALID, "pre-built low-order operator with a non-flux matrix");
    dim3 grid(pl.tiles, pl.tiles, batch);
    femfct_prof_begin(ctx, KC_JACOBI);
    auto go = [&](auto kernel) {
        hipLaunchKernelGGL(kernel, grid, dim3(STRIP_T), 0, ctx->stream, ctx->n, ctx->N, A, Nm, nshared, rhs, rhs_bstride, u_n,
                           u_bstride, ctx->d_ml, dt, ctx->d_L, ctx->d_D, ctx->d_b, ctx->d_xb, ctx->d_part, ctx->d_ctl, pl.K);
    };
    with_constant<8, TILE_HMAX>(pl.H, [&](auto h) {
        constexpr int H = decltype(h)::value;
        with_constant<0, 1>(ctx->tile_lean, [&](auto l) {
            constexpr int LEAN = decltype(l)::value;
            if (pre) go(k_tile_build_jacobi<H, 1, LEAN>); else go(k_tile_build_jacobi<H, 0, LEAN>);
        });
    });
    femfct_prof_end(ctx);
    return FEMFCT_OK;
}

int femfct_enqueue_low_seq(femfct_ctx* ctx, const double* A, double* L, double* D, int32_t entries, double dt) {
    if (!ctx->implicit_cols || ctx->W != 7 || (int64_t)ctx->N * ctx->N != ctx->n || entries < 1 || entries > 65535)
        return femfct_fail(ctx, FEMFCT_ERR_INVALID, "low-order sequence: structured mesh in vertex order only");
    femfct_prof_begin(ctx, KC_ASSEMBLE);
    hipLaunchKernelGGL(k_low_seq, dim3((ctx->n + 255) / 256, entries), dim3(256), 0, ctx->stream, ctx->n, ctx->N, A, ctx->d_ml,
                       dt, L, D);
    femfct_prof_end(ctx);
    return FEMFCT_OK;
}

int femfct_enqueue_tile_jacobi(femfct_ctx* ctx, const TilePlan& pl, const double* L, const double* b, double* xa,
                               double* xb, int launch, int g_build, int32_t batch, bool last, int bn_launch, int defer) {
    const bool big = femfct_tile_big(ctx, pl);
    double* bigp = big ? ctx->d_bigpart : nullptr;
    double* pk = ((last || defer) && !big) ? ctx->d_partk : nullptr;
    dim3 grid(pl.tiles, pl.tiles, batch);
    femfct_prof_begin(ctx, KC_JACOBI);
    auto go = [&](auto kernel, int defer_arg) {
        hipLaunchKernelGGL(kernel, grid, dim3(STRIP_T), 0, ctx->stream, ctx->n, ctx->N, L, b, xa, xb, ctx->d_part, ctx->d_ctl,
                           launch, pl.K, g_build, ctx->rel_tol, bigp, pk, bn_launch, defer_arg);
    };
    with_constant<0, 1>(ctx->tile_lean, [&](auto l) {
        constexpr int LEAN = decltype(l)::value;
        if (big) {
            go(k_tile_jacobi<8, 0, 1, LEAN>, 0);
            femfct_launch_reduce_resid(ctx, (int64_t)pl.tiles * pl.tiles, launch, batch);
        } else {
            with_constant<8, TILE_HMAX>(pl.H, [&](auto h) {
                constexpr int H = decltype(h)::value;
                if (pk && !defer) go(k_tile_jacobi<H, 1, 0, LEAN>, 0); else go(k_tile_jacobi<H, 0, 0, LEAN>, defer);
            });
        }
    });
    femfct_prof_end(ctx);
    return FEMFCT_OK;
}

void femfct_launch_reduce_resid(femfct_ctx* ctx, int64_t count, int launch, int32_t batch) {
    hipLaunchKernelGGL(k_reduce_resid, dim3(batch), dim3(STRIP_T), 0, ctx->stream, ctx->d_bigpart, count, ctx->d_ctl, launch);
}

int femfct_enqueue_tile_dudt_cheb(femfct_ctx* ctx, MatRef A, VecRef rhs, int64_t rhs_bstride, double* ulow,
                                  int budget_units, int part_count, int iters_per_unit, int exact_k, int iters,
                                  const double* omegas, double md_scale, int32_t batch, int* tail_first) {
    constexpr int H = 10;
    const int T = TILE_L - 2 * H, t = (ctx->N + T - 1) / T;
    const int K = std::min(iters - 1, H - 1);
    CheOmegas om;
    for (int k = 0; k < K; ++k) om.w[k] = omegas[k + 1];
    const bool last = (K + 1 == iters);
    double* omid = last ? ctx->d_du : ctx->d_y0;
    double* oold = last ? nullptr : ctx->d_y2;
    femfct_prof_begin(ctx, KC_DUDT_RHS);
    with_constant<0, 1>(ctx->tile_lean, [&](auto l) {
        hipLaunchKernelGGL(k_tile_dudt_cheb<decltype(l)::value>, dim3(t, exact_k < 0 ? t + 1 : t, batch), dim3(STRIP_T), 0,
                           ctx->stream, ctx->n, ctx->N, A, rhs, rhs_bstride, ctx->d_M, ctx->d_xa, ctx->d_xb, ulow, ctx->d_rdu, omid,
                           oold, ctx->d_part, ctx->d_ctl, budget_units, part_count, iters_per_unit, ctx->rel_tol,
                           exact_k ? ctx->d_partk : nullptr, exact_k, K, om, md_scale, omegas[0]);
    });
    femfct_prof_end(ctx);
    if (tail_first) *tail_first = last ? 0 : K + 2;
    if (last || tail_first) return FEMFCT_OK;
    TilePlan tp;
    tp.H = H; tp.K = H; tp.tiles = t;
    return femfct_enqueue_tile_cheb(ctx, tp, ctx->d_rdu, ctx->d_y0, ctx->d_y2, ctx->d_du, K + 2, iters, omegas, md_scale,
                                    ctx->d_y1, ctx->d_rp, ctx->d_y0, ctx->d_y2, batch, nullptr);
}

int femfct_enqueue_tile_cheb(femfct_ctx* ctx, const TilePlan& pl, const double* b, const double* in_mid,
                             const double* in_old, double* y_out, int k_first, int k_last, const double* omegas,
                             double md_scale, double* bufA0, double* bufA1, double* bufB0, double* bufB1, int32_t batch,
                             const ChebIO* io_in) {
    ChebIO io0{};
    if (io_in) io0 = *io_in;
    io0.mid_ref = make_ref(nullptr); io0.mid_bs = 0; io0.out_ref = make_ref(nullptr); io0.out_bs = 0;
    for_cheb_launches(k_first, k_last, pl.K, omegas, in_mid, in_old, y_out, bufA0, bufA1, bufB0, bufB1,
                      [&](int k0, int k1, const CheOmegas& om, const double* mid, const double* old, double* omid, double* oold) {
        femfct_prof_begin(ctx, KC_CHEB);
        ChebIO io = io0;
        io.k0 = k0 - 1;
        if (io_in && k0 == k_first) { io.mid_ref = io_in->mid_ref; io.mid_bs = io_in->mid_bs; }
        if (io_in && k1 == k_last + 1) { io.out_ref = io_in->out_ref; io.out_bs = io_in->out_bs; }
        with_constant<8, TILE_HMAX>(pl.H, [&](auto h) {
            with_constant<0, 1>(ctx->tile_lean, [&](auto l) {
                hipLaunchKernelGGL((k_tile_cheb<decltype(h)::value, decltype(l)::value>), dim3(pl.tiles, pl.tiles, batch),
                                   dim3(STRIP_T), 0, ctx->stream, ctx->n, ctx->N, ctx->d_M, b, mid, old, omid, oold, k1 - k0, om,
                                   md_scale, io);
            });
        });
        femfct_prof_end(ctx);
    });
    return FEMFCT_OK;
}

static EndArgs step_end_args(const femfct_ctx* ctx, int32_t batch, bool fuse_end) {
    EndArgs e{};
    e.level = nullptr;
    if (fuse_end) {
        e.level = ctx->d_level; e.delta = ctx->rep_last ? ctx->end_req_delta * ctx->rep_total : 0;
        e.ord_adv = ctx->rep_last ? ctx->rep_total : 0; e.ord_off = ctx->ord_bias; e.ctl = ctx->d_ctl; e.log = ctx->d_log;
        e.kctl = ctx->end_req_krylov ? (const KrylovCtl*)ctx->d_kry_ctl : nullptr; e.klog = (KrylovCtl*)ctx->d_klog;
        e.batch = batch; e.ticket = ctx->d_ticket;
    }
    return e;
}

int femfct_enqueue_tile_cheb_flux_limit(femfct_ctx* ctx, const double* b, const double* in_mid, const double* in_old,
                                        int k_first, int k_last, const double* omegas, double md_scale, MatRef D,
                                        const double* ulow, double dt, VecRef out, int64_t out_bstride, int32_t batch,
                                        bool fuse_end) {
    const int K = k_last - k_first + 1;
    if (K < 1 || K > 10) return femfct_fail(ctx, FEMFCT_ERR_INVALID, "fused Chebyshev tail: %d iterations", K);
    const EndArgs e = step_end_args(ctx, batch, fuse_end);
    CheOmegas om;
    for (int k = k_first; k <= k_last; ++k) om.w[k - k_first] = omegas[k - 1];
    const int t = (ctx->N + 7) / 8;
    femfct_prof_begin(ctx, KC_FLUX);
    with_constant<0, 1>(femfct_geom_mass(ctx), [&](auto gm) {
        with_constant<0, 1>(ctx->tile_lean, [&](auto l) {
            hipLaunchKernelGGL((k_tile_cheb_flux_limit<decltype(gm)::value, decltype(l)::value>), dim3(t, t, batch), dim3(STRIP_T),
                               0, ctx->stream, ctx->n, ctx->N, ctx->h, ctx->d_M, b, in_mid, in_old, K, om, md_scale, D, ulow,
                               ctx->d_ml, dt, out, out_bstride, e);
        });
    });
    femfct_prof_end(ctx);
    return FEMFCT_OK;
}

int femfct_enqueue_tile_flux_limit(femfct_ctx* ctx, const double* D, const double* ulow, const double* du, double dt,
                                   VecRef out, int64_t out_bstride, int32_t batch, bool* fuse_end_io, int half_d) {
    const bool fuse_end = fuse_end_io && *fuse_end_io && ctx->N <= 512;
    if (fuse_end_io) *fuse_end_io = fuse_end;
    const EndArgs e = step_end_args(ctx, batch, fuse_end);
    femfct_prof_begin(ctx, KC_FLUX);
    const bool geom = femfct_geom_mass(ctx);
    auto go = [&](auto kernel, int PL) {
        const int t = (ctx->N + PL - 2 * FL_H - 1) / (PL - 2 * FL_H);
        hipLaunchKernelGGL(kernel, dim3(t, t, batch), dim3(PL * PL), 0, ctx->stream, ctx->n, ctx->N, ctx->h, ctx->d_M, D, ulow, du,
                           ctx->d_ml, dt, out, out_bstride, e);
    };
    with_constant<0, 1>(geom, [&](auto g) {
        with_constant<0, 1>(half_d != 0, [&](auto hd) {
            constexpr int G = decltype(g)::value, HD = decltype(hd)::value;
            if (ctx->N <= 512) go(k_tile_flux_limit<16, G, HD>, 16); else go(k_tile_flux_limit<32, G, HD>, 32);
        });
    });
    femfct_prof_end(ctx);
    return FEMFCT_OK;
}


bool femfct_geom_mass(const femfct_ctx* ctx) {
    return ctx->geom_mass && ctx->structured && ctx->mass_is_mesh && ctx->implicit_cols;
}

bool femfct_cheb_flux_fusable(const femfct_ctx* ctx, int32_t batch) {
    if (!ctx->fuse_flux || ctx->N > 512) return false;
    const int t = (ctx->N + 7) / 8;
    return (int64_t)t * t * batch <= ctx->wg_slots;
}

bool femfct_tile_plan(const femfct_ctx* ctx, TilePlan* pl, bool need_partials, int budget, int batch) {
    if (!femfct_tiles_usable(ctx)) return false;
    int H = 8;
    const bool small = ctx->N <= 512;
    if (small) {
        if (budget <= 0) H = 10;
        else {
            int best = 1 << 30;
            for (int h = 8; h <= TILE_HMAX; ++h) {
                const int T = TILE_L - 2 * h, t = (ctx->N + T - 1) / T;
                if (h > 10 && (!ctx->deep_halo || (int64_t)t * t * batch > ctx->wg_slots)) break;
                int launches = (budget + h - 1) / h;
                if (launches < best) { best = launches; H = h; }
            }
        }
    }
    if (small && ctx->strip_k >= 8 && ctx->strip_k <= TILE_HMAX) H = ctx->strip_k;
    const int T = TILE_L - 2 * H;
    const int t = (ctx->N + T - 1) / T;
    if (need_partials && (int64_t)t * t > FEMFCT_MAX_PARTIALS) return false;
    if (t > 65535) return false;
    pl->tiles = t;
    pl->K = H;
    pl->H = H;
    return true;
}

bool femfct_tile_big(const femfct_ctx* ctx, const TilePlan& pl) {
    return (int64_t)pl.tiles * pl.tiles > FEMFCT_MAX_PARTIALS;
}
```

fem-fct-pdeco_amd/csrc/traj_common.h:

```cpp
#pragma once

#include <chrono>

#include "femfct_internal.h"
#include "device_utils.h"
#include "forms.h"

#include <algorithm>
#include <stdio.h>
#include <stdlib.h>

int femfct_ensure_traj_ws(femfct_ctx* ctx, int32_t batch, int32_t steps);
int femfct_ensure_krylov_ws(femfct_ctx* ctx, int32_t batch);
int femfct_enqueue_step_end(femfct_ctx* ctx, int delta, int32_t batch, bool with_krylov);
void femfct_request_fused_end(femfct_ctx* ctx, int delta, bool with_krylov);
int femfct_enqueue_step_ref(femfct_ctx* ctx, const double* A, const double* N, int32_t nshared, VecRef rhs,
                            int64_t rhs_bstride, VecRef u_n, int64_t u_bstride, double dt, VecRef u_out,
                            int64_t out_bstride, int32_t batch, int32_t budget);
int femfct_enqueue_step_mat(femfct_ctx* ctx, MatRef A, const double* N, int32_t nshared, VecRef rhs, int64_t rhs_bstride,
                            VecRef u_n, int64_t u_bstride, double dt, VecRef u_out, int64_t out_bstride, int32_t batch,
                            int32_t budget);
int femfct_enqueue_axpby(femfct_ctx* ctx, int64_t count, double alpha, const double* a, double beta, const double* b,
                         double* out);
struct SbOpArgs;
bool femfct_inline_ops_wanted(const femfct_ctx* ctx, int32_t batch);
int femfct_enqueue_step_op(femfct_ctx* ctx, MatRef A, const SbOpArgs* sb, const double* N, int32_t nshared, VecRef rhs,
                           int64_t rhs_bstride, VecRef u_n, int64_t u_bstride, double dt, VecRef u_out, int64_t out_bstride,
                           int32_t batch, int32_t budget);

static inline int femfct_round_kry_budget(const femfct_ctx* ctx, int b) {
    b = (b + 3) & ~3;
    if (b < 4) b = 4;
    if (b > ctx->kry_max_iters) b = ctx->kry_max_iters;
    return b;
}

template <class F>
int femfct_run_graph_reps(femfct_ctx* ctx, femfct_ctx::GraphKey key, int reps, int delta, F&& enqueue_one) {
    key.push_back(key_bits((int32_t)reps));
    key.push_back(key_bits((int32_t)ctx->pair_rows));
    key.push_back(key_bits((int32_t)ctx->solver));
    key.push_back(key_bits(ctx->low_src));
    key.push_back(key_bits(ctx->low_dt));
    key.push_back(key_bits((int32_t)ctx->tile_lean));
    struct Restore {
        femfct_ctx* c;
        ~Restore() { c->level_bias = 0; c->ord_bias = 0; c->rep_total = 1; c->rep_last = true; }
    } restore{ctx};
    return femfct_run_graph(ctx, key, [&]() {
        for (int r = 0; r < reps; ++r) {
            ctx->level_bias = r * delta; ctx->ord_bias = r; ctx->rep_total = reps; ctx->rep_last = (r == reps - 1);
            int rc = enqueue_one();
            if (rc != FEMFCT_OK) return rc;
        }
        return (int)FEMFCT_OK;
    });
}

static inline VecRef lref(const femfct_ctx* ctx, const double* p, const int32_t* level, int64_t stride, int32_t off) {
    return make_ref(p, level, stride, off + (level ? ctx->level_bias : 0));
}

struct SweepSpec {
    SweepKind kind;
    int32_t num_steps, batch;
    int level0;
    bool krylov;
    bool full_rows;
};
struct SweepPlan {
    int budget, kbudget;
    bool meshp, cheb;
};
enum { FEMFCT_SWEEP_REPEAT = -1 };
FEMFCT_INTERNAL int femfct_sweep_plan(femfct_ctx* ctx, const SweepSpec& sp, SweepPlan* plan);
FEMFCT_INTERNAL int femfct_sweep_fetch_logs(femfct_ctx* ctx, const SweepSpec& sp);
FEMFCT_INTERNAL int femfct_sweep_verdict(femfct_ctx* ctx, const SweepSpec& sp, const SweepPlan& plan);
FEMFCT_INTERNAL void femfct_sweep_report_times(const SweepSpec& sp, const double t[4]);

static inline int femfct_next_kry_budget(const femfct_ctx* ctx, int worst, bool cheb) {
    return std::min(ctx->kry_max_iters, cheb ? std::max(8, worst + 1) : std::max(8, worst + worst / 4 + 2));
}

template <class Begin, class Step>
int femfct_run_sweep(femfct_ctx* ctx, const SweepSpec& sp, Begin&& begin, Step&& step) {
    struct RestoreSolver {
        femfct_ctx* c;
        ~RestoreSolver() { c->solver = c->solver_user; c->pair_rows = false; }
    } restore_solver{ctx};
    const bool dbg_t = getenv("FEMFCT_DEBUG_TIMES") != nullptr;
    auto now = []() { return std::chrono::duration<double, std::milli>(std::chrono::steady_clock::now().time_since_epoch()).count(); };
    for (;;) {
        SweepPlan plan;
        int rc = femfct_sweep_plan(ctx, sp, &plan);
        if (rc != FEMFCT_OK) return rc;
        double t[4] = {dbg_t ? now() : 0.0, 0.0, 0.0, 0.0};
        if ((rc = begin()) != FEMFCT_OK) return rc;
        if (dbg_t) t[1] = now();
        int32_t init[2] = {sp.level0, 0};
        HIP_TRY(ctx, hipMemcpyAsync(ctx->d_level, init, sizeof init, hipMemcpyHostToDevice, ctx->stream));
        const int32_t per_graph = std::max(1, std::min(ctx->steps_per_graph, sp.num_steps));
        for (int32_t k = 0; k < sp.num_steps; k += per_graph) {
            rc = step(plan.budget, plan.kbudget, std::min(per_graph, sp.num_steps - k));
            if (rc != FEMFCT_OK) return rc;
        }
        if (dbg_t) t[2] = now();
        if ((rc = femfct_sweep_fetch_logs(ctx, sp)) != FEMFCT_OK) return rc;
        if (dbg_t) { t[3] = now(); femfct_sweep_report_times(sp, t); }
        rc = femfct_sweep_verdict(ctx, sp, plan);
        if (rc != FEMFCT_SWEEP_REPEAT) return rc;
    }
}
```

Before: 31250 timesteps/s.

## Add fitted smaller tile patches and hex-cone loading for tiled Chebyshev kernels

Adds a 'fit' mode, on by default, that launches the dudt-Cheb and Cheb-flux-limit kernels with smaller patches (26 and 30 wide, stepping 6 nodes per tile). Block sizes are rounded to the wavefront, so the grid still fits in the workgroup-slot budget for this mesh. Also adds an opt-in 'cone' mode that uses hexagonal distance so only nodes inside the dependency cone load matrix rows and vectors, plus tuning-only timestamp instrumentation. The intent is to spread work over more CUs with less redundant halo load per workgroup, at the cost of more recomputed halo overall and spare threads in partial wavefronts.

```diff
diff --git a/fem-fct-pdeco_amd/csrc/ctx.hip b/fem-fct-pdeco_amd/csrc/ctx.hip
--- a/fem-fct-pdeco_amd/csrc/ctx.hip
+++ b/fem-fct-pdeco_amd/csrc/ctx.hip
@@ -260,6 +260,8 @@
     if (const char* e = getenv("FEMFCT_FUSE_FLUX")) ctx->fuse_flux = atoi(e) != 0;
     if (const char* e = getenv("FEMFCT_FUSE_DUDT")) ctx->fuse_dudt = atoi(e) != 0;
     if (const char* e = getenv("FEMFCT_TILE_LEAN")) ctx->tile_lean = atoi(e) != 0;
+    if (const char* e = getenv("FEMFCT_TILE_CONE")) ctx->tile_cone = atoi(e) != 0;
+    if (const char* e = getenv("FEMFCT_TILE_FIT")) ctx->tile_fit = atoi(e) != 0;
     if (const char* e = getenv("FEMFCT_FUSE_END")) ctx->fuse_end = atoi(e) != 0;
     if (const char* e = getenv("FEMFCT_TILE4")) ctx->tile4_mode = atoi(e);
     if (const char* e = getenv("FEMFCT_LMASK")) ctx->l_mask = atoi(e) != 0;
@@ -395,6 +397,9 @@
         hipFree(ctx->d_pair_trace);
         ctx->d_pair_trace = nullptr;
     }
+#ifdef FEMFCT_TUNING
+    if (const char* path = getenv("FEMFCT_TILE_TRACE")) femfct_tile_phase_dump(path);
+#endif
     femfct_release_pattern(ctx);
     hipStreamDestroy(ctx->stream);
     delete ctx;
diff --git a/fem-fct-pdeco_amd/csrc/femfct_internal.h b/fem-fct-pdeco_amd/csrc/femfct_internal.h
--- a/fem-fct-pdeco_amd/csrc/femfct_internal.h
+++ b/fem-fct-pdeco_amd/csrc/femfct_internal.h
@@ -123,6 +123,8 @@
     bool fuse_flux = true;
     bool fuse_dudt = true;
     int tile_lean = 1;
+    int tile_cone = 0;
+    int tile_fit = 1;
     bool exact_iters = false;
     int32_t bandwidth = 0;
     int32_t strip_k = 0;
@@ -257,6 +259,10 @@
 bool femfct_tile_plan(const femfct_ctx* ctx, TilePlan* pl, bool need_partials = true, int budget = 0, int batch = 1);
 bool femfct_tile_big(const femfct_ctx* ctx, const TilePlan& pl);
 bool femfct_cheb_flux_fusable(const femfct_ctx* ctx, int32_t batch);
+bool femfct_tile_fit(const femfct_ctx* ctx, int32_t batch);
+#ifdef FEMFCT_TUNING
+void femfct_tile_phase_dump(const char* path);
+#endif
 bool femfct_geom_mass(const femfct_ctx* ctx);
 int femfct_enqueue_tile_build_jacobi(femfct_ctx* ctx, const TilePlan& pl, struct MatRef A, const double* Nm, int32_t nshared,
                                      struct VecRef rhs, int64_t rhs_bstride, struct VecRef u_n, int64_t u_bstride, double dt,
diff --git a/fem-fct-pdeco_amd/csrc/kernels_tile32.hip b/fem-fct-pdeco_amd/csrc/kernels_tile32.hip
--- a/fem-fct-pdeco_amd/csrc/kernels_tile32.hip
+++ b/fem-fct-pdeco_amd/csrc/kernels_tile32.hip
@@ -14,6 +14,22 @@
 #define TILE_HMAX 13
 
 namespace {
+
+#ifdef FEMFCT_TUNING
+__device__ unsigned long long g_tile_phase[4][4];
+#define TILE_STAMP_BEGIN()                                                                                              \
+    unsigned long long ts0_ = 0, ts1_ = 0;                                                                              \
+    const bool ts_on_ = threadIdx.x == 0 && blockIdx.z == 0 && blockIdx.x == gridDim.x / 2 && blockIdx.y == gridDim.x / 2; \
+    if (ts_on_) ts0_ = __builtin_amdgcn_s_memrealtime()
+#define TILE_STAMP_LOADED() do { if (ts_on_) { __builtin_amdgcn_s_waitcnt(0); ts1_ = __builtin_amdgcn_s_memrealtime(); } } while (0)
+#define TILE_STAMP_END(id) do { if (ts_on_) {                                                                           \
+        const unsigned long long ts2_ = __builtin_amdgcn_s_memrealtime();                                               \
+        g_tile_phase[id][0] += ts1_ - ts0_; g_tile_phase[id][1] += ts2_ - ts0_; g_tile_phase[id][2] += 1; } } while (0)
+#else
+#define TILE_STAMP_BEGIN() do { } while (0)
+#define TILE_STAMP_LOADED() do { } while (0)
+#define TILE_STAMP_END(id) do { } while (0)
+#endif
 
 struct TileGeom {
     int lx, ly, gx, gy, i;
@@ -49,14 +65,38 @@
         int nx = min(max(g.lx + dx[s], 0), PL - 1), ny = min(max(g.ly + dy[s], 0), PL - 1);
         g.nb[s] = ny * PLD + nx;
     }
+    if (PL * PL % WAVE != 0 && threadIdx.x >= PL * PL) {
+        g.inside = g.owned = false;
+        g.i = 0;
+        g.kvalid = 0;
+        g.self = 0;
+    }
     return g;
 }
 
-template <int H>
+template <int PL>
+__device__ __forceinline__ bool tile_spare() {
+    return PL * PL % WAVE != 0 && threadIdx.x >= PL * PL;
+}
+
+template <int H, int PL = TILE_L>
 __device__ __forceinline__ int tile_dist(const TileGeom& g) {
-    constexpr int T = TILE_L - 2 * H;
+    constexpr int T = PL - 2 * H;
     const int ddx = max(max(H - g.lx, g.lx - (H + T - 1)), 0), ddy = max(max(H - g.ly, g.ly - (H + T - 1)), 0);
     return max(ddx, ddy);
+}
+
+template <int H, int PL = TILE_L>
+__device__ __forceinline__ int tile_hexdist(const TileGeom& g) {
+    constexpr int T = PL - 2 * H;
+    const int ex = g.lx - min(max(g.lx, H), H + T - 1), ey = g.ly - min(max(g.ly, H), H + T - 1);
+    return max(max(abs(ex), abs(ey)), abs(ex - ey));
+}
+
+template <int H, int LEAN, int PL = TILE_L>
+__device__ __forceinline__ int lean_dist(const TileGeom& g) {
+    if constexpr (LEAN == 2) return tile_hexdist<H, PL>(g);
+    else return tile_dist<H, PL>(g);
 }
 
 struct LeanAddr {
@@ -64,7 +104,8 @@
     double* me0;
 };
 
-__device__ __forceinline__ LeanAddr lean_addr(double (*bufs)[TILE_L * TILE_LD], const TileGeom& g) {
+template <int PL>
+__device__ __forceinline__ LeanAddr lean_addr(double (*bufs)[PL * (PL + 1)], const TileGeom& g) {
     LeanAddr a;
     a.me0 = &bufs[0][g.self];
 #pragma unroll
@@ -104,10 +145,10 @@
     return xo;
 }
 
-template <int BUF>
+template <int BUF, int PL = TILE_L>
 __device__ __forceinline__ void lean_cheb_iter(const LeanAddr& a, bool live, const double* mv, double md, double rmd, double bv,
                                                double wk, double& ym, double& yo) {
-    constexpr int RD = BUF * TILE_L * TILE_LD, WR = (1 - BUF) * TILE_L * TILE_LD;
+    constexpr int RD = BUF * PL * (PL + 1), WR = (1 - BUF) * PL * (PL + 1);
     if (live) {
         double acc = md * ym;
 #pragma unroll
@@ -180,11 +221,23 @@
     const double* L = L_ + moff;
     const double* xin = ((launch & 1) ? xb_ : xa_) + voff;
     double* xout = ((launch & 1) ? xa_ : xb_) + voff;
+    TILE_STAMP_BEGIN();
     const TileGeom g = tile_geom<TILE_L - 2 * H, H>(N);
+    constexpr bool CONE = LEAN == 2;
     double lv[W - 1], dg = 1.0, rdg = 1.0, bv = 0.0, xi = 0.0;
 #pragma unroll
     for (int s = 0; s < W - 1; ++s) lv[s] = 0.0;
-    if (g.inside) {
+    if constexpr (CONE) {
+        const int dist = tile_hexdist<H>(g);
+        if (g.inside && ((dist < K && g.kvalid > 0) || g.owned)) {
+            dg = L[g.i];
+            rdg = 1.0 / dg;
+#pragma unroll
+            for (int s = 1; s < W; ++s) lv[s - 1] = L[(int64_t)s * n + g.i];
+            bv = b_[voff + g.i];
+        }
+        if (g.inside && dist <= K) xi = xin[g.i];
+    } else if (g.inside) {
         dg = L[g.i];
         rdg = 1.0 / dg;
 #pragma unroll
@@ -195,11 +248,12 @@
     xs[0][g.self] = xi;
     if (LEAN) xs[1][g.self] = xi;
     __syncthreads();
+    TILE_STAMP_LOADED();
     double rmax = 0.0;
     int cur = 0;
     [[maybe_unused]] double xo = xi;
-    [[maybe_unused]] const int klive = min(g.kvalid, K - tile_dist<H>(g));
-    [[maybe_unused]] const LeanAddr a = lean_addr(xs, g);
+    [[maybe_unused]] const int klive = min(g.kvalid, K - lean_dist<H, LEAN>(g));
+    [[maybe_unused]] const LeanAddr a = lean_addr<TILE_L>(xs, g);
     if (!EXACT) {
         if constexpr (LEAN) xo = lean_jacobi(a, klive, K, g.owned, lv, dg, rdg, bv, xi, rmax);
         else
@@ -273,6 +327,7 @@
         else if (defer) partk[((int64_t)bz * 16 + launch) * FEMFCT_MAX_PARTIALS + wg] = rmax;
         else p[(launch & 1) * FEMFCT_MAX_PARTIALS + wg] = rmax;
     }
+    TILE_STAMP_END(1);
 }
 
 template <int H, int PRE, int LEAN>
@@ -300,25 +355,45 @@
     const double* rhs = vec_ptr(rhs_ref);
     if (rhs) rhs += bz * rhs_bstride;
     const double* u = vec_ptr(u_ref) + bz * u_bstride;
+    TILE_STAMP_BEGIN();
     const TileGeom g = tile_geom<TILE_L - 2 * H, H>(N);
     double lv[W - 1], dv[W - 1], dsum = 0.0, rs = 0.0;
     double dg = 1.0, rdg = 1.0, bv = 0.0, xi = 0.0;
     if constexpr (PRE) {
 #pragma unroll
         for (int s = 0; s < W - 1; ++s) lv[s] = 0.0;
-        if (g.inside) {
-            dg = A[g.i];
-#pragma unroll
-            for (int s = 1; s < W; ++s) lv[s - 1] = A[(int64_t)s * n + g.i];
-        }
-#pragma unroll
-        for (int s = 0; s < W - 1; ++s) rs += lv[s];
-        if (g.inside) {
-            const double mli = ml[g.i];
-            rs += dg;
-            rdg = 1.0 / dg;
-            xi = u[g.i];
-            bv = mli * xi + (rhs ? dt * rhs[g.i] : 0.0);
+        if constexpr (LEAN == 2) {
+            const int dist = tile_hexdist<H>(g);
+            const bool row = g.inside && ((dist < K && g.kvalid > 0) || g.owned);
+            if (row) {
+                dg = A[g.i];
+#pragma unroll
+                for (int s = 1; s < W; ++s) lv[s - 1] = A[(int64_t)s * n + g.i];
+            }
+#pragma unroll
+            for (int s = 0; s < W - 1; ++s) rs += lv[s];
+            if (g.inside && dist <= K) xi = u[g.i];
+            if (row) {
+                const double mli = ml[g.i];
+                rs += dg;
+                rdg = 1.0 / dg;
+                bv = mli * xi + (rhs ? dt * rhs[g.i] : 0.0);
+            }
+        } else {
+            if (g.inside) {
+                dg = A[g.i];
+#pragma unroll
+                for (int s = 1; s < W; ++s) lv[s - 1] = A[(int64_t)s * n + g.i];
+            }
+#pragma unroll
+            for (int s = 0; s < W - 1; ++s) rs += lv[s];
+            if (g.inside) {
+                const double mli = ml[g.i];
+                rs += dg;
+                rdg = 1.0 / dg;
+                xi = u[g.i];
+                bv = mli * xi + (rhs ? dt * rhs[g.i] : 0.0);
+            }
         }
     } else {
         const int dx[6] = {1, 1, 0, -1, -1, 0}, dy[6] = {0, 1, 1, 0, -1, -1};
@@ -388,10 +463,11 @@
     xs[0][g.self] = xi;
     if (LEAN) xs[1][g.self] = xi;
     __syncthreads();
+    TILE_STAMP_LOADED();
     double rmax = 0.0;
     int cur = 0;
     [[maybe_unused]] double xo = xi;
-    if constexpr (LEAN) xo = lean_jacobi(lean_addr(xs, g), min(g.kvalid, K - tile_dist<H>(g)), K, g.owned, lv, dg, rdg, bv, xi, rmax);
+    if constexpr (LEAN) xo = lean_jacobi(lean_addr<TILE_L>(xs, g), min(g.kvalid, K - lean_dist<H, LEAN>(g)), K, g.owned, lv, dg, rdg, bv, xi, rmax);
     else
     for (int k = 0; k < K; ++k) {
         const double* c = xs[cur];
@@ -414,6 +490,7 @@
         p[2 * FEMFCT_MAX_PARTIALS + wg] = bmax;
         p[3 * FEMFCT_MAX_PARTIALS + wg] = rsmin;
     }
+    TILE_STAMP_END(0);
 }
 
 __global__ void __launch_bounds__(256)
@@ -477,10 +554,22 @@
     if (cio.mid_ref.base) ymid_ = vec_ptr(cio.mid_ref) + (int64_t)blockIdx.z * cio.mid_bs - voff;
     if (cio.out_ref.base) omid_ = const_cast<double*>(vec_ptr(cio.out_ref)) + (int64_t)blockIdx.z * cio.out_bs - voff;
     const TileGeom g = tile_geom<TILE_L - 2 * H, H>(N);
+    constexpr bool CONE = LEAN == 2;
     double mv[W - 1], md = 1.0, rmd = 1.0, bv = 0.0, ym = 0.0, yo = 0.0;
 #pragma unroll
     for (int s = 0; s < W - 1; ++s) mv[s] = 0.0;
-    if (g.inside) {
+    if constexpr (CONE) {
+        const int dist = tile_hexdist<H>(g);
+        if (g.inside && ((dist < K && g.kvalid > 0) || g.owned)) {
+            md = M[g.i];
+            rmd = 1.0 / (md_scale * md);
+#pragma unroll
+            for (int s = 1; s < W; ++s) mv[s - 1] = M[(int64_t)s * n + g.i];
+            bv = b_[voff + g.i];
+            if (yold_) yo = yold_[voff + g.i];
+        }
+        if (g.inside && dist <= K && ymid_) ym = ymid_[voff + g.i];
+    } else if (g.inside) {
         md = M[g.i];
         rmd = 1.0 / (md_scale * md);
 #pragma unroll
@@ -493,8 +582,8 @@
         ys[0][g.self] = ym;
         ys[1][g.self] = ym;
         __syncthreads();
-        const int klive = min(g.kvalid, K - tile_dist<H>(g));
-        const LeanAddr a = lean_addr(ys, g);
+        const int klive = min(g.kvalid, K - lean_dist<H, LEAN>(g));
+        const LeanAddr a = lean_addr<TILE_L>(ys, g);
         int k = 0;
         for (; k + 1 < K; k += 2) {
             lean_cheb_iter<0>(a, k < klive, mv, md, rmd, bv, omd ? omd[k] : om.w[k], ym, yo);
@@ -620,23 +709,50 @@
     if (FL_L == 16) step_end_by_last_workgroup(e);
 }
 
-template <int GEOM, int LEAN>
-__global__ void __launch_bounds__(STRIP_T, LEAN ? 8 : 1)
+template <int GEOM, int LEAN, int PL>
+__global__ void __launch_bounds__((PL * PL + WAVE - 1) / WAVE * WAVE, (LEAN && PL == TILE_L) ? 8 : 1)
 k_tile_cheb_flux_limit(int n, int N, double h, const double* __restrict__ M, const double* __restrict__ b_,
                        const double* __restrict__ ymid_, const double* __restrict__ yold_, int K, CheOmegas om,
                        double md_scale, MatRef D_ref, const double* __restrict__ ulow_,
                        const double* __restrict__ ml, double dt, VecRef out_ref, int64_t out_bstride, EndArgs e) {
-    constexpr int W = 7, HH = 12;
-    __shared__ double ys[LEAN ? 2 : 3][TILE_L * TILE_LD];
-    __shared__ double su[TILE_L * TILE_LD], srp[TILE_L * TILE_LD], srm[TILE_L * TILE_LD];
+    constexpr int W = 7, HH = 12, PLD = PL + 1;
+    constexpr bool CONE = LEAN == 2;
+    static_assert(PL == TILE_L || LEAN, "fitted patches run the lean loops only");
+    __shared__ double ys[LEAN ? 2 : 3][PL * PLD];
+    __shared__ double su[PL * PLD], srp[PL * PLD], srm[PL * PLD];
     const int bz = blockIdx.z;
     const int64_t voff = (int64_t)bz * n;
     const double* D_ = mat_ptr(D_ref, bz);
-    const TileGeom g = tile_geom<TILE_L - 2 * HH, HH>(N);
+    TILE_STAMP_BEGIN();
+    const TileGeom g = tile_geom<PL - 2 * HH, HH, PL>(N);
     double mv[W - 1], dv[W - 1], md = 1.0, rmd = 1.0, bv = 0.0, ym = 0.0, yo = 0.0, ui = 0.0, mli = 1.0;
 #pragma unroll
     for (int s = 0; s < W - 1; ++s) { mv[s] = 0.0; dv[s] = 0.0; }
-    if (g.inside) {
+    [[maybe_unused]] bool flux_node = false;
+    if constexpr (CONE) {
+        const int dist = tile_hexdist<HH, PL>(g);
+        flux_node = g.inside && g.kvalid >= K + 1 && dist <= 1;
+        if (g.inside && (min(g.kvalid, K - max(dist - 2, 0)) > 0 || flux_node)) {
+            md = M[g.i];
+            rmd = 1.0 / (md_scale * md);
+            if (GEOM) {
+                const int pc = mass_edge_counts(g.gx, g.gy, N - 1);
+                const double mq = (0.5 * h * h) / 12.0;
+#pragma unroll
+                for (int s = 1; s < W; ++s) mv[s - 1] = (double)((pc >> (2 * (s - 1))) & 3) * mq;
+            } else {
+#pragma unroll
+                for (int s = 1; s < W; ++s) mv[s - 1] = M[(int64_t)s * n + g.i];
+            }
+            bv = b_[voff + g.i];
+            yo = yold_[voff + g.i];
+        }
+        if (g.inside && max(dist - 2, 0) <= K) ym = ymid_[voff + g.i];
+        if (g.inside && dist <= 2) {
+            ui = ulow_[voff + g.i];
+            mli = ml[g.i];
+        }
+    } else if (g.inside) {
         md = M[g.i];
         rmd = 1.0 / (md_scale * md);
         if (GEOM) {
@@ -654,28 +770,31 @@
         ui = ulow_[voff + g.i];
         mli = ml[g.i];
     }
-    ys[0][g.self] = LEAN ? ym : yo;
-    ys[1][g.self] = ym;
-    su[g.self] = ui;
-    srp[g.self] = 1.0;
-    srm[g.self] = 1.0;
+    if (!tile_spare<PL>()) {
+        ys[0][g.self] = LEAN ? ym : yo;
+        ys[1][g.self] = ym;
+        su[g.self] = ui;
+        srp[g.self] = 1.0;
+        srm[g.self] = 1.0;
+    }
     __syncthreads();
+    TILE_STAMP_LOADED();
     step_log_early(e);
-    if (g.inside) {
+    if (g.inside && (!CONE || flux_node)) {
 #pragma unroll
         for (int s = 1; s < W; ++s) dv[s - 1] = D_[(int64_t)s * n + g.i];
     }
     int io = 0, im = 1, in_ = 2;
-    const bool have = g.inside && g.kvalid >= K + 1 && (!LEAN || tile_dist<HH>(g) <= 1);
+    const bool have = g.inside && g.kvalid >= K + 1 && (!LEAN || lean_dist<HH, LEAN, PL>(g) <= 1);
     if constexpr (LEAN) {
-        const int klive = min(g.kvalid, K - max(tile_dist<HH>(g) - 2, 0));
-        const LeanAddr a = lean_addr(ys, g);
+        const int klive = min(g.kvalid, K - max(lean_dist<HH, LEAN, PL>(g) - 2, 0));
+        const LeanAddr a = lean_addr<PL>(ys, g);
         int k = 0;
         for (; k + 1 < K; k += 2) {
-            lean_cheb_iter<0>(a, k < klive, mv, md, rmd, bv, om.w[k], ym, yo);
-            lean_cheb_iter<1>(a, k + 1 < klive, mv, md, rmd, bv, om.w[k + 1], ym, yo);
-        }
-        if (k < K) lean_cheb_iter<0>(a, k < klive, mv, md, rmd, bv, om.w[k], ym, yo);
+            lean_cheb_iter<0, PL>(a, k < klive, mv, md, rmd, bv, om.w[k], ym, yo);
+            lean_cheb_iter<1, PL>(a, k + 1 < klive, mv, md, rmd, bv, om.w[k + 1], ym, yo);
+        }
+        if (k < K) lean_cheb_iter<0, PL>(a, k < klive, mv, md, rmd, bv, om.w[k], ym, yo);
         im = K & 1;
     } else
     for (int k = 0; k < K; ++k) {
@@ -728,19 +847,22 @@
         double* out = const_cast<double*>(vec_ptr(out_ref)) + bz * out_bstride;
         out[g.i] = ui + dt * fbar / mli;
     }
+    TILE_STAMP_END(3);
     step_end_by_last_workgroup(e);
 }
 
-template <int LEAN>
-__global__ void __launch_bounds__(STRIP_T)
-k_tile_dudt_cheb(int n, int N, MatRef A_ref, VecRef rhs_ref, int64_t rhs_bstride,
+template <int LEAN, int GEOM, int PL>
+__global__ void __launch_bounds__((PL * PL + WAVE - 1) / WAVE * WAVE)
+k_tile_dudt_cheb(int n, int N, double h, MatRef A_ref, VecRef rhs_ref, int64_t rhs_bstride,
                  const double* __restrict__ M, const double* __restrict__ xa_, const double* __restrict__ xb_,
                  double* __restrict__ ulow_, double* __restrict__ rdu_, double* __restrict__ omid_,
                  double* __restrict__ oold_, double* __restrict__ part, StepCtl* __restrict__ ctl_, int budget,
                  int part_count, int iters_per_unit, double rel_tol, const double* __restrict__ partk, int exact_k,
                  int K, CheOmegas om, double md_scale, double omega1) {
-    constexpr int W = 7, H = 10;
-    __shared__ double ys[LEAN ? 2 : 3][TILE_L * TILE_LD];
+    constexpr int W = 7, H = 10, PLD = PL + 1;
+    constexpr bool CONE = LEAN == 2;
+    static_assert(PL == TILE_L || LEAN, "fitted patches run the lean loops only");
+    __shared__ double ys[LEAN ? 2 : 3][PL * PLD];
     __shared__ double smem[64];
     const int bz = blockIdx.z;
     StepCtl* ctl = ctl_ + bz;
@@ -761,27 +883,60 @@
     const double* x = (parity ? xb_ : xa_) + voff;
     const double* rhs = vec_ptr(rhs_ref);
     if (rhs) rhs += bz * rhs_bstride;
-    const TileGeom g = tile_geom<TILE_L - 2 * H, H>(N);
+    TILE_STAMP_BEGIN();
+    const TileGeom g = tile_geom<PL - 2 * H, H, PL>(N);
     double av[W], mv[W - 1], md = 1.0, rmd = 1.0, ui = 0.0, ri = 0.0;
 #pragma unroll
     for (int s = 0; s < W; ++s) av[s] = 0.0;
 #pragma unroll
     for (int s = 0; s < W - 1; ++s) mv[s] = 0.0;
-    if (g.inside) {
+    bool need_r = g.kvalid >= 1;
+    if constexpr (CONE) {
+        const int dist = tile_hexdist<H, PL>(g);
+        need_r = need_r && dist <= K;
+        if (g.inside && need_r) {
+            md = M[g.i];
+            rmd = 1.0 / (md_scale * md);
+#pragma unroll
+            for (int s = 0; s < W; ++s) av[s] = A[(int64_t)s * n + g.i];
+            ri = rhs ? rhs[g.i] : 0.0;
+        }
+        if (g.inside && g.kvalid > 1 && dist < K) {
+            if (GEOM) {
+                const int pc = mass_edge_counts(g.gx, g.gy, N - 1);
+                const double mq = (0.5 * h * h) / 12.0;
+#pragma unroll
+                for (int s = 1; s < W; ++s) mv[s - 1] = (double)((pc >> (2 * (s - 1))) & 3) * mq;
+            } else {
+#pragma unroll
+                for (int s = 1; s < W; ++s) mv[s - 1] = M[(int64_t)s * n + g.i];
+            }
+        }
+        if (g.inside && dist <= K + 1) ui = x[g.i];
+    } else if (g.inside) {
         md = M[g.i];
         rmd = 1.0 / (md_scale * md);
 #pragma unroll
         for (int s = 0; s < W; ++s) av[s] = A[(int64_t)s * n + g.i];
-#pragma unroll
-        for (int s = 1; s < W; ++s) mv[s - 1] = M[(int64_t)s * n + g.i];
+        if (GEOM) {
+            const int pc = mass_edge_counts(g.gx, g.gy, N - 1);
+            const double mq = (0.5 * h * h) / 12.0;
+#pragma unroll
+            for (int s = 1; s < W; ++s) mv[s - 1] = (double)((pc >> (2 * (s - 1))) & 3) * mq;
+        } else {
+#pragma unroll
+            for (int s = 1; s < W; ++s) mv[s - 1] = M[(int64_t)s * n + g.i];
+        }
         ui = x[g.i];
         ri = rhs ? rhs[g.i] : 0.0;
     }
     constexpr int UB = LEAN ? 0 : 2;
-    ys[UB][g.self] = ui;
+    const bool spare = tile_spare<PL>();
+    if (!spare) ys[UB][g.self] = ui;
     __syncthreads();
+    TILE_STAMP_LOADED();
     double r = 0.0, y1 = 0.0;
-    if (g.kvalid >= 1) {
+    if (need_r) {
         double acc = av[0] * ui;
 #pragma unroll
         for (int s = 1; s < W; ++s) acc = fma(av[s], ys[UB][g.nb[s - 1]], acc);
@@ -789,25 +944,26 @@
         y1 = omega1 * (r / (md_scale * md));
     }
     if constexpr (LEAN) {
-        ys[1][g.self] = y1;
+        if (!spare) ys[1][g.self] = y1;
         __syncthreads();
-        ys[0][g.self] = y1;
+        if (!spare) ys[0][g.self] = y1;
         double ym = y1, yo = 0.0;
-        const int dist = tile_dist<H>(g);
-        const LeanAddr a = lean_addr(ys, g);
+        const int dist = lean_dist<H, LEAN, PL>(g);
+        const LeanAddr a = lean_addr<PL>(ys, g);
         auto live = [&](int k) { return k + 1 < g.kvalid && k < K - dist; };
         int k = 0;
         for (; k + 1 < K; k += 2) {
-            lean_cheb_iter<1>(a, live(k), mv, md, rmd, r, om.w[k], ym, yo);
-            lean_cheb_iter<0>(a, live(k + 1), mv, md, rmd, r, om.w[k + 1], ym, yo);
-        }
-        if (k < K) lean_cheb_iter<1>(a, live(k), mv, md, rmd, r, om.w[k], ym, yo);
+            lean_cheb_iter<1, PL>(a, live(k), mv, md, rmd, r, om.w[k], ym, yo);
+            lean_cheb_iter<0, PL>(a, live(k + 1), mv, md, rmd, r, om.w[k + 1], ym, yo);
+        }
+        if (k < K) lean_cheb_iter<1, PL>(a, live(k), mv, md, rmd, r, om.w[k], ym, yo);
         if (g.owned) {
             ulow_[voff + g.i] = ui;
             rdu_[voff + g.i] = r;
             omid_[voff + g.i] = ym;
             if (oold_) oold_[voff + g.i] = yo;
         }
+        TILE_STAMP_END(2);
         return;
     }
     __syncthreads();
@@ -837,10 +993,30 @@
         omid_[voff + g.i] = ys[im][g.self];
         if (oold_) oold_[voff + g.i] = ys[io][g.self];
     }
-}
-
-}
-
+    TILE_STAMP_END(2);
+}
+
+}
+
+#ifdef FEMFCT_TUNING
+void femfct_tile_phase_dump(const char* path) {
+    static const char* names[4] = {"k_tile_build_jacobi", "k_tile_jacobi", "k_tile_dudt_cheb", "k_tile_cheb_flux_limit"};
+    unsigned long long h[4][4];
+    if (hipMemcpyFromSymbol(h, HIP_SYMBOL(g_tile_phase), sizeof(h)) != hipSuccess) return;
+    if (FILE* f = fopen(path, "a")) {
+        for (int k = 0; k < 4; ++k)
+            if (h[k][2])
+                fprintf(f, "%-24s launches %8llu  load phase %7.3f us  whole kernel %7.3f us  share %5.1f %%\n", names[k], h[k][2],
+                        0.01 * h[k][0] / h[k][2], 0.01 * h[k][1] / h[k][2], 100.0 * h[k][0] / (double)h[k][1]);
+        fclose(f);
+    }
+    memset(h, 0, sizeof(h));
+    hipMemcpyToSymbol(HIP_SYMBOL(g_tile_phase), h, sizeof(h));
+}
+#endif
+
+
+static int tile_lean_mode(const femfct_ctx* ctx) { return ctx->tile_lean ? (ctx->tile_cone ? 2 : 1) : 0; }
 
 int femfct_enqueue_tile_build_jacobi(femfct_ctx* ctx, const TilePlan& pl, MatRef A, const double* Nm, int32_t nshared,
                                      VecRef rhs, int64_t rhs_bstride, VecRef u_n, int64_t u_bstride, double dt,
@@ -854,7 +1030,7 @@
     };
     with_constant<8, TILE_HMAX>(pl.H, [&](auto h) {
         constexpr int H = decltype(h)::value;
-        with_constant<0, 1>(ctx->tile_lean, [&](auto l) {
+        with_constant<0, 2>(tile_lean_mode(ctx), [&](auto l) {
             constexpr int LEAN = decltype(l)::value;
             if (pre) go(k_tile_build_jacobi<H, 1, LEAN>); else go(k_tile_build_jacobi<H, 0, LEAN>);
         });
@@ -884,7 +1060,7 @@
         hipLaunchKernelGGL(kernel, grid, dim3(STRIP_T), 0, ctx->stream, ctx->n, ctx->N, L, b, xa, xb, ctx->d_part, ctx->d_ctl,
                            launch, pl.K, g_build, ctx->rel_tol, bigp, pk, bn_launch, defer_arg);
     };
-    with_constant<0, 1>(ctx->tile_lean, [&](auto l) {
+    with_constant<0, 2>(tile_lean_mode(ctx), [&](auto l) {
         constexpr int LEAN = decltype(l)::value;
         if (big) {
             go(k_tile_jacobi<8, 0, 1, LEAN>, 0);
@@ -909,6 +1085,8 @@
                                   const double* omegas, double md_scale, int32_t batch, int* tail_first) {
     constexpr int H = 10;
     const int T = TILE_L - 2 * H, t = (ctx->N + T - 1) / T;
+    const bool fit = femfct_tile_fit(ctx, batch);
+    const int tl = fit ? (ctx->N + 5) / 6 : t;
     const int K = std::min(iters - 1, H - 1);
     CheOmegas om;
     for (int k = 0; k < K; ++k) om.w[k] = omegas[k + 1];
@@ -916,11 +1094,21 @@
     double* omid = last ? ctx->d_du : ctx->d_y0;
     double* oold = last ? nullptr : ctx->d_y2;
     femfct_prof_begin(ctx, KC_DUDT_RHS);
-    with_constant<0, 1>(ctx->tile_lean, [&](auto l) {
-        hipLaunchKernelGGL(k_tile_dudt_cheb<decltype(l)::value>, dim3(t, exact_k < 0 ? t + 1 : t, batch), dim3(STRIP_T), 0,
-                           ctx->stream, ctx->n, ctx->N, A, rhs, rhs_bstride, ctx->d_M, ctx->d_xa, ctx->d_xb, ulow, ctx->d_rdu, omid,
-                           oold, ctx->d_part, ctx->d_ctl, budget_units, part_count, iters_per_unit, ctx->rel_tol,
+    auto go = [&](auto kernel, int PL) {
+        hipLaunchKernelGGL(kernel, dim3(tl, exact_k < 0 ? tl + 1 : tl, batch), dim3((PL * PL + WAVE - 1) / WAVE * WAVE), 0,
+                           ctx->stream, ctx->n, ctx->N, ctx->h, A, rhs, rhs_bstride, ctx->d_M, ctx->d_xa, ctx->d_xb, ulow, ctx->d_rdu,
+                           omid, oold, ctx->d_part, ctx->d_ctl, budget_units, part_count, iters_per_unit, ctx->rel_tol,
                            exact_k ? ctx->d_partk : nullptr, exact_k, K, om, md_scale, omegas[0]);
+    };
+    with_constant<0, 1>(ctx->tile_lean && femfct_geom_mass(ctx), [&](auto gm) {
+        constexpr int GM = decltype(gm)::value;
+        if (fit) {
+            if (ctx->tile_cone) go(k_tile_dudt_cheb<2, GM, 26>, 26); else go(k_tile_dudt_cheb<1, GM, 26>, 26);
+        } else if constexpr (GM) {
+            if (ctx->tile_cone) go(k_tile_dudt_cheb<2, 1, TILE_L>, TILE_L); else go(k_tile_dudt_cheb<1, 1, TILE_L>, TILE_L);
+        } else {
+            with_constant<0, 2>(tile_lean_mode(ctx), [&](auto l) { go(k_tile_dudt_cheb<decltype(l)::value, 0, TILE_L>, TILE_L); });
+        }
     });
     femfct_prof_end(ctx);
     if (tail_first) *tail_first = last ? 0 : K + 2;
@@ -946,7 +1134,7 @@
         if (io_in && k0 == k_first) { io.mid_ref = io_in->mid_ref; io.mid_bs = io_in->mid_bs; }
         if (io_in && k1 == k_last + 1) { io.out_ref = io_in->out_ref; io.out_bs = io_in->out_bs; }
         with_constant<8, TILE_HMAX>(pl.H, [&](auto h) {
-            with_constant<0, 1>(ctx->tile_lean, [&](auto l) {
+            with_constant<0, 2>(tile_lean_mode(ctx), [&](auto l) {
                 hipLaunchKernelGGL((k_tile_cheb<decltype(h)::value, decltype(l)::value>), dim3(pl.tiles, pl.tiles, batch),
                                    dim3(STRIP_T), 0, ctx->stream, ctx->n, ctx->N, ctx->d_M, b, mid, old, omid, oold, k1 - k0, om,
                                    md_scale, io);
@@ -978,14 +1166,20 @@
     const EndArgs e = step_end_args(ctx, batch, fuse_end);
     CheOmegas om;
     for (int k = k_first; k <= k_last; ++k) om.w[k - k_first] = omegas[k - 1];
-    const int t = (ctx->N + 7) / 8;
+    const bool fit = femfct_tile_fit(ctx, batch);
+    const int t = fit ? (ctx->N + 5) / 6 : (ctx->N + 7) / 8;
     femfct_prof_begin(ctx, KC_FLUX);
+    auto go = [&](auto kernel, int PL) {
+        hipLaunchKernelGGL(kernel, dim3(t, t, batch), dim3((PL * PL + WAVE - 1) / WAVE * WAVE), 0, ctx->stream, ctx->n, ctx->N,
+                           ctx->h, ctx->d_M, b, in_mid, in_old, K, om, md_scale, D, ulow, ctx->d_ml, dt, out, out_bstride, e);
+    };
     with_constant<0, 1>(femfct_geom_mass(ctx), [&](auto gm) {
-        with_constant<0, 1>(ctx->tile_lean, [&](auto l) {
-            hipLaunchKernelGGL((k_tile_cheb_flux_limit<decltype(gm)::value, decltype(l)::value>), dim3(t, t, batch), dim3(STRIP_T),
-                               0, ctx->stream, ctx->n, ctx->N, ctx->h, ctx->d_M, b, in_mid, in_old, K, om, md_scale, D, ulow,
-                               ctx->d_ml, dt, out, out_bstride, e);
-        });
+        constexpr int GM = decltype(gm)::value;
+        if (fit) {
+            if (ctx->tile_cone) go(k_tile_cheb_flux_limit<GM, 2, 30>, 30); else go(k_tile_cheb_flux_limit<GM, 1, 30>, 30);
+        } else {
+            with_constant<0, 2>(tile_lean_mode(ctx), [&](auto l) { go(k_tile_cheb_flux_limit<GM, decltype(l)::value, TILE_L>, TILE_L); });
+        }
     });
     femfct_prof_end(ctx);
     return FEMFCT_OK;
@@ -1024,6 +1218,12 @@
     return (int64_t)t * t * batch <= ctx->wg_slots;
 }
 
+bool femfct_tile_fit(const femfct_ctx* ctx, int32_t batch) {
+    if (!ctx->tile_lean || !ctx->tile_fit) return false;
+    const int t = (ctx->N + 5) / 6;
+    return (int64_t)t * (t + 1) * batch <= ctx->wg_slots;
+}
+
 bool femfct_tile_plan(const femfct_ctx* ctx, TilePlan* pl, bool need_partials, int budget, int batch) {
     if (!femfct_tiles_usable(ctx)) return false;
     int H = 8;
diff --git a/fem-fct-pdeco_amd/csrc/traj_common.h b/fem-fct-pdeco_amd/csrc/traj_common.h
--- a/fem-fct-pdeco_amd/csrc/traj_common.h
+++ b/fem-fct-pdeco_amd/csrc/traj_common.h
@@ -42,7 +42,7 @@
     key.push_back(key_bits((int32_t)ctx->solver));
     key.push_back(key_bits(ctx->low_src));
     key.push_back(key_bits(ctx->low_dt));
-    key.push_back(key_bits((int32_t)ctx->tile_lean));
+    key.push_back(key_bits((int32_t)(ctx->tile_lean | ctx->tile_cone << 1 | ctx->tile_fit << 2)));
     struct Restore {
         femfct_ctx* c;
         ~Restore() { c->level_bias = 0; c->ord_bias = 0; c->rep_total = 1; c->rep_last = true; }
```

Result: faster. 33440 timesteps/s (median of 6 runs) (+7.0%).
